# hmc-lair-shark-tracking/auv-sim

Measured on NVIDIA B200. Metric: edge_evals_per_s, higher is better.
Workload: dtype f32

## Files before the change

auv-sim_b200/csrc/edge.cuh:

```cuda
#pragma once
#include "geom.cuh"

#ifndef AUV_EDGE_ONE
#define AUV_EDGE_ONE 0
#endif

namespace auv {

template <typename R> struct SteerParams {
    R d2e, dmax, neg_dmax, freq, min_dist, two_vel;
    R w_diff, o_dist, o_diff, o_vel;
};

template <int G> struct Log2 { static const int v = (G == 32) ? 5 : (G == 16) ? 4 : (G == 8) ? 3 : (G == 4) ? 2 : 1; };

template <typename R, int G, bool FLAT = true> struct GroupScratch {
    R us[FLAT ? 3 * G : 32];
    R wx[G + 1], wy[G + 1];
    unsigned char jmp[FLAT ? Log2<G>::v : 1][FLAT ? 3 * G + 4 : 4];
};

template <typename R> struct EdgeOut {
    R x, y, th, t, len;
    int nwp;
    int n_exp;
    uint32_t ctr;
    int status;
    bool safe;
    R s2; uint32_t cnt; uint64_t mask;
    R self_s2; int self_hab; bool leaf_moved;
};

__device__ __forceinline__ float sinc_small(float h) {
    float z = h * h;
    if (z > 0.25f) {
        float sn, cs;
        Ar<float, false>::sincos(h, &sn, &cs);
        return __fdividef(sn, h);
    }
    float p = fmaf(z, 2.7557319e-6f, -1.9841270e-4f);
    p = fmaf(z, p, 8.3333333e-3f);
    p = fmaf(z, p, -1.6666667e-1f);
    return fmaf(z, p, 1.0f);
}

template <typename R, int G, bool DO_COLLIDE, bool DO_COST, bool WRITE_WP, bool FLAT = false, bool ONE_CHUNK = false, bool GRIDS = false>
__device__ __forceinline__ void eval_edge(const Grp<G> &g, GroupScratch<R, G, FLAT> &sc, const EnvView<R> &env,
                                          const Stream<R> &rng, uint32_t ctr, const SteerParams<R> &sp,
                                          R px, R py, R pth, R pt, R plen, R w3, int n_hab,
                                          R *wp_out, int wp_cap, EdgeOut<R> &out) {
    typedef typename Policy<R>::A A;
    const bool VERIFY = Policy<R>::VERIFY;
    const int LOG = Log2<G>::v;

    R u0 = rng.u(ctr);
    ctr += 1;
    int n_exp = (int)A::floor(uniform_ab<R>((R)0, sp.freq, u0));
    out.n_exp = n_exp;
    out.status = 0;

    R cth = pth, cx = px, cy = py, ct = pt, clen = plen;
    R csin = 0, ccos = 0;
    if (VERIFY) A::sincos(pth, &csin, &ccos);
    int nwp = 1;
    bool hit = false, outside = false, zero_div = false, moved = false, degenerate = false, parent_clear = false, parent_many = false;
    R acc_s2 = 0; uint32_t acc_cnt = 0; uint64_t acc_mask = 0;
    R self_s2 = 0; int self_hab = -1;

    if (DO_COLLIDE) {
        if (g.gl == 0) { sc.wx[G] = px; sc.wy[G] = py; }
        const Cls pcl = env.template classify<GRIDS>(px, py);
        parent_clear = (pcl.code & 4u) != 0u;
        parent_many = (pcl.code & AUV_GRID_CIRC_MANY) != 0u;
        if (VERIFY || !AUV_EDGE_ONE || (pcl.code & AUV_GRID_SLOW)) {
            outside = !point_within_c<R>(env, pcl, px, py);
            if (!parent_clear && !parent_many) hit = point_hits_circles_c<R>(env, pcl, px, py);
        } else outside = point_unsafe_one<R>(env, pcl.code, px, py);
    }

    for (int base = 0; base < n_exp; base += G) {
        const int nact = min(G, n_exp - base);
        const bool act = g.gl < nact;
        R dist = 0, diff = 0, vt = 1;
        bool valid = false;
        if (FLAT) {
    #pragma unroll
            for (int r = 0; r < 3; r++) {
                int s = g.gl + G * r;
                sc.us[s] = (s < 3 * nact) ? rng.u(ctr + (uint32_t)s) : (R)0;
            }
            g.sync();
    #pragma unroll
            for (int r = 0; r < 3; r++) {
                int s = g.gl + G * r;
                int nx = 3 * G;
                if (s <= 3 * G - 3) {
                    R dist = uniform_ab<R>((R)0, sp.d2e, sc.us[s]);
                    R diff = uniform_ab<R>(sp.neg_dmax, sp.dmax, sc.us[s + 1]);
                    nx = s + 2 + (A::fabs(dist) > A::fabs(diff) ? 1 : 0);
                    if (nx > 3 * G) nx = 3 * G;
                }
                sc.jmp[0][s] = (unsigned char)nx;
            }
            if (g.gl == 0) {
    #pragma unroll
                for (int d = 0; d < LOG; d++) sc.jmp[d][3 * G] = (unsigned char)(3 * G);
            }
            g.sync();
    #pragma unroll
            for (int d = 1; d < LOG; d++) {
    #pragma unroll
                for (int r = 0; r < 3; r++) {
                    int s = g.gl + G * r;
                    sc.jmp[d][s] = sc.jmp[d - 1][sc.jmp[d - 1][s]];
                }
                g.sync();
            }
            int o = 0;
    #pragma unroll
            for (int d = 0; d < LOG; d++)
                if ((g.gl >> d) & 1) o = sc.jmp[d][o];
            if (act) {
                dist = uniform_ab<R>((R)0, sp.d2e, sc.us[o]);
                diff = uniform_ab<R>(sp.neg_dmax, sp.dmax, sc.us[o + 1]);
                valid = A::fabs(dist) > A::fabs(diff);
                if (valid) vt = uniform_ab<R>((R)0, sp.two_vel, sc.us[o + 2]);
            }
            int o_end = g.bcast(o + 2 + (valid ? 1 : 0), nact - 1);
            ctr += (uint32_t)o_end;

        } else {
            if (act) {
                const uint32_t p0 = ctr + 3u * (uint32_t)g.gl;
                dist = uniform_ab<R>((R)0, sp.d2e, rng.u(p0));
                diff = uniform_ab<R>(sp.neg_dmax, sp.dmax, rng.u(p0 + 1u));
                valid = A::fabs(dist) > A::fabs(diff);
                if (valid) vt = uniform_ab<R>((R)0, sp.two_vel, rng.u(p0 + 2u));
            }
            ctr += 3u * (uint32_t)nact;
        }
        R phi = 0, radius = 0, chord = 0;
        if (valid) {
            if (VERIFY) {
                R s1 = A::add(dist, diff), s2 = A::sub(dist, diff);
                R den = A::add(-s1, s2);
                R num = A::add(s1, s2);
                if (den == (R)0) zero_div = true;
                radius = A::div(num, den);
                R r2 = A::mul((R)2, radius);
                if (r2 == (R)0) zero_div = true;
                phi = A::div(num, r2);
            } else {
                if (diff == (R)0) zero_div = true;
                phi = -diff;
                chord = dist * sinc_small((float)diff * 0.5f);
            }
            if (vt == (R)0) zero_div = true;
        }
        R th;
        if (VERIFY) th = (R)grp_scan_serial<G>(g, (double)phi, (double)cth);
        else th = grp_scan_incl<G>(g, phi) + cth;
        R dx = 0, dy = 0, movement = 0, dt = 0;
        if (VERIFY) {
            R s1v, c1v;
            A::sincos(th, &s1v, &c1v);
            R s0v = g.up(s1v, 1), c0v = g.up(c1v, 1);
            if (g.gl == 0) { s0v = csin; c0v = ccos; }
            if (valid) {
                dx = A::mul(radius, A::sub(s1v, s0v));
                dy = A::mul(radius, A::add(-c1v, c0v));
                movement = A::sqrt(A::sq2(dx, dy));
                dt = A::div(movement, vt);
            }
            csin = g.bcast(s1v, G - 1); ccos = g.bcast(c1v, G - 1);
        } else {
            if (valid) {
                R sm, cm;
                A::sincos(th - (R)0.5 * phi, &sm, &cm);
                dx = chord * cm; dy = chord * sm;
                movement = chord;
                dt = A::div(movement, vt);
            }
        }
        R x, y, t, len;
        if (VERIFY) {
            x = (R)grp_scan_serial<G>(g, (double)dx, (double)cx);
            y = (R)grp_scan_serial<G>(g, (double)dy, (double)cy);
            t = (R)grp_scan_serial<G>(g, (double)dt, (double)ct);
            len = (R)grp_scan_serial<G>(g, (double)movement, (double)clen);
        } else {
            x = grp_scan_incl<G>(g, dx) + cx;
            y = grp_scan_incl<G>(g, dy) + cy;
            t = grp_scan_incl<G>(g, dt) + ct;
            len = grp_scan_incl<G>(g, movement) + clen;
        }
        const bool is_wp = valid && (movement >= sp.min_dist);
        const unsigned wpm = g.ballot(is_wp);
        const unsigned vm = g.ballot(valid);
        if (vm) moved = true;
        const int last_valid = vm ? 31 - __clz(vm) : -1;

        if (WRITE_WP) {
            if (is_wp) {
                int row = nwp - 1 + __popc(wpm & ((1u << g.gl) - 1u));
                if (row < wp_cap) {
                    R *w = wp_out + 6 * (size_t)row;
                    w[0] = x; w[1] = y; w[2] = th; w[3] = vt; w[4] = t; w[5] = len;
                }
            }
        }
        Cls cl; cl.code = AUV_GRID_ALL_AMBIG | 4u; cl.idx = -1;
        if ((DO_COLLIDE || DO_COST) && (is_wp || g.gl == last_valid)) cl = env.template classify<GRIDS>(x, y);
        if (DO_COLLIDE) {
            bool in = true, h1 = false;
            if (is_wp) {
                if (VERIFY || !AUV_EDGE_ONE) {
                    in = point_within_c<R>(env, cl, x, y);
                    if (!(cl.code & AUV_GRID_CIRC_MANY)) h1 = point_hits_circles_c<R>(env, cl, x, y);
                } else {
                    in = !point_unsafe_one<R>(env, cl.code, x, y);
                    if (__builtin_expect((cl.code & AUV_GRID_SLOW) != 0u, 0)) {
                        in = point_within_c<R>(env, cl, x, y);
                        if (!(cl.code & AUV_GRID_CIRC_MANY)) h1 = point_hits_circles_c<R>(env, cl, x, y);
                    }
                }
            }
            if (g.ballot(!in)) outside = true;
            if (g.ballot(h1)) hit = true;
            const bool circles_needed = g.ballot(is_wp && !(cl.code & 4u) && (cl.code & AUV_GRID_CIRC_MANY)) != 0u ||
                                        (base == 0 && !parent_clear && parent_many);
            if (env.K > 0 && circles_needed && !outside) {
                if (is_wp) { int slot = __popc(wpm & ((1u << g.gl) - 1u)); sc.wx[slot] = x; sc.wy[slot] = y; }
                g.sync();
                const int nw = __popc(wpm);
                bool h = false;
#pragma unroll 1
                for (int k = g.gl; k < env.K; k += G) {
                    R ccx = env.cx[k], ccy = env.cy[k];
                    R q = A::inf();
                    if (base == 0) q = A::sq2(A::sub(sc.wx[G], ccx), A::sub(sc.wy[G], ccy));
#pragma unroll 1
                    for (int j = 0; j < nw; j++) {
                        R qq = A::sq2(A::sub(sc.wx[j], ccx), A::sub(sc.wy[j], ccy));
                        q = qq < q ? qq : q;
                    }
                    if (VERIFY) h = h || (A::sqrt(q) <= env.creff[k]);
                    else h = h || (q <= env.creff2[k]);
                }
                if (g.ballot(h)) hit = true;
                g.sync();
            }
        }
        if (DO_COST) {
            const bool need = is_wp || (g.gl == last_valid);
            Contrib c; c.bin = -1; c.cell = -1; c.hab = -1;
            if (need) c = point_contrib<R>(env, x, y, t, 0xffffffffu, n_hab, cl);
            R ps2 = (R)0;
            if (c.bin >= 0 && c.cell >= 0) ps2 = A::mul(w3, env.probs[(size_t)c.bin * env.C + c.cell]);
            const bool counts = is_wp && c.bin >= 0;
            acc_s2 += grp_sum<G>(g, counts ? ps2 : (R)0);
            unsigned hm = g.ballot(counts && c.hab >= 0);
            acc_cnt += __popc(hm);
            unsigned long long mbits = (counts && c.hab >= 0) ? (1ull << c.hab) : 0ull;
            if (G == 32) {
                const unsigned lo = __reduce_or_sync(0xffffffffu, (unsigned)mbits), hi = __reduce_or_sync(0xffffffffu, (unsigned)(mbits >> 32));
                mbits = ((unsigned long long)hi << 32) | lo;
            } else {
#pragma unroll
                for (int m = G / 2; m > 0; m >>= 1) mbits |= g.xorv(mbits, m);
            }
            acc_mask |= mbits;
            if (last_valid >= 0) {
                self_s2 = g.bcast((c.bin >= 0) ? ps2 : (R)0, last_valid);
                self_hab = g.bcast((c.bin >= 0) ? c.hab : -1, last_valid);
            }
        }
        nwp += __popc(wpm);
        if (last_valid >= 0) {
            cth = g.bcast(th, last_valid); cx = g.bcast(x, last_valid); cy = g.bcast(y, last_valid);
            ct = g.bcast(t, last_valid); clen = g.bcast(len, last_valid);
        }
        g.sync();
        if (g.ballot(zero_div)) {
            if (VERIFY) out.status = 2; else degenerate = true;
            break;
        }
        if (ONE_CHUNK) break;
    }
    if (DO_COLLIDE && n_exp == 0 && env.K > 0 && !parent_clear && parent_many) {
        bool h = false;
#pragma unroll 1
        for (int k = g.gl; k < env.K; k += G) {
            R q = A::sq2(A::sub(px, env.cx[k]), A::sub(py, env.cy[k]));
            if (VERIFY) h = h || (A::sqrt(q) <= env.creff[k]);
            else h = h || (q <= env.creff2[k]);
        }
        if (g.ballot(h)) hit = true;
    }
    if (!rng.consumed_ok(ctr)) out.status = 4;
    out.x = cx; out.y = cy; out.th = cth; out.t = ct; out.len = clen;
    out.nwp = nwp; out.ctr = ctr;
    out.safe = !(hit || outside || degenerate);
    out.s2 = acc_s2; out.cnt = acc_cnt; out.mask = acc_mask;
    out.self_s2 = self_s2; out.self_hab = self_hab; out.leaf_moved = moved;
}

}
```

auv-sim_b200/csrc/env.cuh:

```cuda
#pragma once
#include "common.cuh"

namespace auv {

struct EnvHeader {
    int K, E, H, T, C, NB, NP, NCAND;
    int convex;
    int hot_bytes;
    int total_bytes;
    int off_cx, off_cy, off_cr, off_creff, off_creff2;
    int off_px, off_py;
    int off_hx, off_hy, off_hr, off_hr2;
    int off_b0, off_b1;
    int off_brk, off_piece, off_c1, off_cell;
    int off_probs;
    int off_xb;
    int nxb;
    int off_pfirst;
    int off_grid;
    int gnx, gny;
    int bins_uniform;
    int off_one;
    int pad_;
    double bbox[4];
    double gx0, gy0, gs;
    double bin_s0, bin_w;
    double xb0, xbw;
    double pad2_[2];
};
static_assert(sizeof(EnvHeader) % 16 == 0, "EnvHeader must keep 16-byte alignment of the arrays");

#define AUV_GRID_HAB_NONE 128u
#define AUV_GRID_HAB_AMBIG 192u
#define AUV_GRID_HAB_ONE 64u
#define AUV_GRID_CIRC_MANY (1u << 11)
#define AUV_GRID_HAB_MANY (1u << 12)
#define AUV_GRID_POLY_FULL (1u << 13)
#define AUV_GRID_CIRC_ONE (1u << 14)
#define AUV_GRID_POLY_ONE (1u << 15)
#define AUV_GRID_SLOW (1u << 31)
#define AUV_GRID_ALL_AMBIG ((AUV_GRID_HAB_AMBIG << 3) | AUV_GRID_CIRC_MANY | AUV_GRID_HAB_MANY | AUV_GRID_POLY_FULL | AUV_GRID_SLOW)

struct Cls { unsigned code; int idx; };

template <typename R> struct alignas(8) PFirst { R c1; int v; };

template <typename R> struct alignas(16) One { R x, y, z, w; };

template <typename R> struct EnvView {
    int K, E, H, T, C, NB, NP, convex;
    int gnx, gny, ncell, bins_uniform, nxb;
    R gx0, gy0, ginv, gxo, gyo, bin_s0, bin_w, bin_winv, bin_off, bin_lo, bin_hi, xb0, xbinv, xbo;
    const unsigned *grid;
    const unsigned *grid0s;
    const PFirst<R> *pfirst;
    const One<R> *cone, *pone, *hone;
    const EnvView<R> *shared_self;
    const unsigned short *xb;
    R minx, miny, maxx, maxy;
    const R *cx, *cy, *cr, *creff, *creff2;
    const R *px, *py;
    const R *hx, *hy, *hr, *hr2;
    const R *b0, *b1;
    const R *brk;
    const int *piece;
    const R *c1;
    const int *cell;
    const R *probs;

    __device__ __forceinline__ void bind(const unsigned char *hot, const unsigned char *probs_base) {
        const EnvHeader *h = (const EnvHeader *)hot;
        K = h->K; E = h->E; H = h->H; T = h->T; C = h->C; NB = h->NB; NP = h->NP; convex = h->convex;
        shared_self = nullptr;
        minx = (R)h->bbox[0]; miny = (R)h->bbox[1]; maxx = (R)h->bbox[2]; maxy = (R)h->bbox[3];
        cx = (const R *)(hot + h->off_cx); cy = (const R *)(hot + h->off_cy);
        cr = (const R *)(hot + h->off_cr); creff = (const R *)(hot + h->off_creff);
        creff2 = (const R *)(hot + h->off_creff2);
        px = (const R *)(hot + h->off_px); py = (const R *)(hot + h->off_py);
        hx = (const R *)(hot + h->off_hx); hy = (const R *)(hot + h->off_hy);
        hr = (const R *)(hot + h->off_hr); hr2 = (const R *)(hot + h->off_hr2);
        b0 = (const R *)(hot + h->off_b0); b1 = (const R *)(hot + h->off_b1);
        brk = (const R *)(hot + h->off_brk); piece = (const int *)(hot + h->off_piece);
        c1 = (const R *)(hot + h->off_c1); cell = (const int *)(hot + h->off_cell);
        probs = (const R *)(probs_base + h->off_probs);
        pfirst = (const PFirst<R> *)(hot + h->off_pfirst);
        cone = (const One<R> *)(hot + h->off_one); pone = cone + (K + 1); hone = pone + (E > 0 ? E : 1);
        bin_lo = T > 0 ? b0[0] : (R)1; bin_hi = T > 0 ? b1[T - 1] : (R)0;
    }
    __device__ __forceinline__ void assume_hot_shared(bool probs_too) const {
        __builtin_assume(__isShared(cx)); __builtin_assume(__isShared(cy)); __builtin_assume(__isShared(cr));
        __builtin_assume(__isShared(creff)); __builtin_assume(__isShared(creff2));
        __builtin_assume(__isShared(px)); __builtin_assume(__isShared(py));
        __builtin_assume(__isShared(hx)); __builtin_assume(__isShared(hy)); __builtin_assume(__isShared(hr));
        __builtin_assume(__isShared(hr2)); __builtin_assume(__isShared(b0)); __builtin_assume(__isShared(b1));
        __builtin_assume(__isShared(brk)); __builtin_assume(__isShared(piece)); __builtin_assume(__isShared(c1));
        __builtin_assume(__isShared(cell)); __builtin_assume(__isShared(pfirst)); __builtin_assume(__isShared(xb));
        __builtin_assume(__isShared(cone)); __builtin_assume(__isShared(pone)); __builtin_assume(__isShared(hone));
        if (probs_too) __builtin_assume(__isShared(probs));
    }
    __device__ __forceinline__ void bind_grid(const unsigned char *blob_global, const unsigned char *hot) {
        const EnvHeader *h = (const EnvHeader *)hot;
        gnx = h->gnx; gny = h->gny; bins_uniform = h->bins_uniform; nxb = h->nxb;
        xb0 = (R)h->xb0; xbinv = (R)(1.0 / h->xbw); xbo = (R)(-h->xb0 / h->xbw); xb = (const unsigned short *)(hot + h->off_xb);
        gx0 = (R)h->gx0; gy0 = (R)h->gy0; ginv = (R)(1.0 / h->gs);
        gxo = (R)(-h->gx0 / h->gs); gyo = (R)(-h->gy0 / h->gs);
        bin_s0 = (R)h->bin_s0; bin_w = (R)h->bin_w; bin_winv = (R)(1.0 / h->bin_w); bin_off = (R)(-h->bin_s0 / h->bin_w);
        grid = (const unsigned *)(blob_global + h->off_grid);
        grid0s = nullptr;
        ncell = gnx * gny;
    }
    template <bool GRIDS = false>
    __device__ __forceinline__ Cls classify(R x, R y) const {
        Cls c;
        int ix, iy;
        if (sizeof(R) == 4) {
            const float fx = fmaf((float)x, (float)ginv, (float)gxo), fy = fmaf((float)y, (float)ginv, (float)gyo);
            ix = __float_as_int(__fadd_rd(fx, 8388608.f)) - 0x4B000000;
            iy = __float_as_int(__fadd_rd(fy, 8388608.f)) - 0x4B000000;
        } else {
            const R fx = (x - gx0) * ginv, fy = (y - gy0) * ginv;
            const bool in = fx >= (R)0 && fy >= (R)0 && fx < (R)gnx && fy < (R)gny;
            ix = in ? (int)fx : -1; iy = in ? (int)fy : -1;
        }
        if (!((unsigned)ix < (unsigned)gnx && (unsigned)iy < (unsigned)gny)) {
            c.code = gnx > 0 ? (((AUV_GRID_HAB_AMBIG << 3) | AUV_GRID_HAB_MANY | AUV_GRID_CIRC_MANY | AUV_GRID_POLY_FULL) | 2u) : AUV_GRID_ALL_AMBIG;
            c.idx = -1; return c;
        }
        c.idx = iy * gnx + ix;
        c.code = GRIDS ? grid0s[c.idx] : __ldg(grid + c.idx);
        return c;
    }
    __device__ __forceinline__ unsigned word1(const Cls &c) const { return __ldg(grid + ncell + c.idx); }
    __device__ __forceinline__ unsigned word2(const Cls &c) const { return __ldg(grid + 2 * ncell + c.idx); }
};

__device__ __forceinline__ uint32_t smem_u32(const void *p) {
    return (uint32_t)__cvta_generic_to_shared(p);
}
__device__ __forceinline__ void mbar_init(uint64_t *bar, int count) {
    asm volatile("mbarrier.init.shared::cta.b64 [%0], %1;" ::"r"(smem_u32(bar)), "r"(count));
    asm volatile("fence.mbarrier_init.release.cluster;" ::: "memory");
}
__device__ __forceinline__ void mbar_expect_tx(uint64_t *bar, uint32_t bytes) {
    asm volatile("mbarrier.arrive.expect_tx.shared::cta.b64 _, [%0], %1;" ::"r"(smem_u32(bar)), "r"(bytes)
                 : "memory");
}
__device__ __forceinline__ void tma_bulk_g2s(void *dst, const void *src, uint32_t bytes, uint64_t *bar) {
    asm volatile(
        "cp.async.bulk.shared::cluster.global.mbarrier::complete_tx::bytes [%0], [%1], %2, [%3];" ::"r"(
            smem_u32(dst)),
        "l"(src), "r"(bytes), "r"(smem_u32(bar))
        : "memory");
}
__device__ __forceinline__ void mbar_wait(uint64_t *bar, uint32_t phase) {
    asm volatile(
        "{\n"
        ".reg .pred p;\n"
        "WAIT_%=:\n"
        "mbarrier.try_wait.parity.shared::cta.b64 p, [%0], %1;\n"
        "@p bra DONE_%=;\n"
        "bra WAIT_%=;\n"
        "DONE_%=:\n"
        "}\n" ::"r"(smem_u32(bar)),
        "r"(phase)
        : "memory");
}

__device__ __forceinline__ void stage_env_tma(unsigned char *smem_dst, const unsigned char *blob,
                                              int bytes, uint64_t *bar) {
    if (threadIdx.x == 0) mbar_init(bar, 1);
    __syncthreads();
    if (threadIdx.x == 0) {
        mbar_expect_tx(bar, (uint32_t)bytes);
        for (int o = 0; o < bytes; o += 65536) {
            int n = bytes - o < 65536 ? bytes - o : 65536;
            tma_bulk_g2s(smem_dst + o, blob + o, (uint32_t)n, bar);
        }
    }
    mbar_wait(bar, 0);
}

struct EnvStagePlan { int bytes; int probs_staged; };

}
```

auv-sim_b200/csrc/plan.cu:

```cuda
#include <stdlib.h>
#include "plan_common.cuh"
#include "dubins.cuh"

#ifndef AUV_PLAN_PREFETCH
#define AUV_PLAN_PREFETCH 0
#endif

namespace auv {

#define AUV_LAUNCH_CHECK2()                                                                 \
    do {                                                                                    \
        g_launches++;                                                                       \
        cudaError_t e_ = cudaGetLastError();                                                \
        if (e_ != cudaSuccess)                                                              \
            return set_err(AUVRRT_ERR_CUDA, "%s:%d launch: %s", __FILE__, __LINE__,         \
                           cudaGetErrorString(e_));                                         \
    } while (0)

#ifndef AUV_PLAN_THREADS32
#define AUV_PLAN_THREADS32 896
#endif
#ifndef AUV_PLAN_MINB32
#define AUV_PLAN_MINB32 (896 / AUV_PLAN_THREADS32)
#endif
template <typename R, int G> struct PlanCta {
    static const int T = (sizeof(R) == 4 && G == 32) ? AUV_PLAN_THREADS32 : 128, MINB = (sizeof(R) == 4 && G == 32) ? AUV_PLAN_MINB32 : 7;
};

struct WsLayout {
    size_t slot_bytes;
    size_t rows, xy, pool, next, head, tail, count;
};

template <typename R> static WsLayout make_layout(int cap, int nb, int nchunks) {
    WsLayout L;
    size_t o = 0;
    auto take = [&](size_t bytes) { size_t r = o; o += (bytes + 127) & ~(size_t)127; return r; };
    L.rows = take(sizeof(NodeRow<R>) * (size_t)cap);
    L.xy = take(2 * sizeof(R) * (size_t)cap);
    L.pool = take(4 * 32 * (size_t)nchunks); L.next = take(4 * (size_t)nchunks);
    L.head = take(4 * (size_t)(nb + 2)); L.tail = take(4 * (size_t)(nb + 2)); L.count = take(4 * (size_t)(nb + 2));
    L.slot_bytes = o;
    return L;
}

template <typename R> struct Tree {
    NodeRow<R> *row;
    R *nx, *ny;
    int *pool, *next, *head, *tail, *count;
    __device__ __forceinline__ void bind(unsigned char *b, const WsLayout &L, int cap) {
        row = (NodeRow<R> *)(b + L.rows);
        nx = (R *)(b + L.xy); ny = nx + cap;
        pool = (int *)(b + L.pool); next = (int *)(b + L.next);
        head = (int *)(b + L.head); tail = (int *)(b + L.tail); count = (int *)(b + L.count);
    }
};

template <typename R> struct DubinsEdge {
    bool ok;
    bool safe;
    R x, y, th, t, len;
    R s2; uint32_t cnt; unsigned long long mask;
    R self_s2; int self_hab;
};
template <typename R>
__device__ __forceinline__ void dubins_edge_eval(const EnvView<R> &env, const PlanP<R> &P, R px, R py, R pth, R pt, R plen,
                                                 R sx, R sy, R sth, bool do_tests, R *rows, int room, DubinsEdge<R> &e) {
    typedef typename Policy<R>::A A;
    e.ok = false; e.safe = false; e.x = px; e.y = py; e.th = pth; e.t = pt; e.len = plen;
    e.s2 = 0; e.cnt = 0; e.mask = 0ull; e.self_s2 = 0; e.self_hab = -1;
    const DubinsPath<R> d = dubins_shortest<R>(px, py, pth, sx, sy, sth, P.rho);
    if (d.word < 0) return;
    e.ok = true;
    const R s_end = d.length < P.eta ? d.length : P.eta;
    const R step = A::div(s_end, (R)(P.W - 1));
    DubinsSampler<R> smp;
    smp.init(d, px, py, pth, P.rho);
    bool bad = false;
    if (do_tests) {
        const Cls pcl = env.classify(px, py);
        bad = point_unsafe_c<R>(env, pcl, px, py);
    }
#pragma unroll 1
    for (int k = 1; k < P.W; k++) {
        const R sk = A::mul((R)k, step);
        R x, y, th;
        smp.at(sk, x, y, th);
        const R t = A::add(pt, A::div(sk, P.vel)), len = A::add(plen, sk);
        if (do_tests) {
            const Cls cl = env.classify(x, y);
            bad = bad || point_unsafe_c<R>(env, cl, x, y);
            const Contrib c = point_contrib<R>(env, x, y, t, 0xffffffffu, env.H, cl);
            const R ps2 = (c.bin >= 0 && c.cell >= 0) ? A::mul(P.w3, env.probs[(size_t)c.bin * env.C + c.cell]) : (R)0;
            if (c.bin >= 0) {
                e.s2 = A::add(e.s2, ps2);
                if (c.hab >= 0) { e.cnt++; e.mask |= 1ull << c.hab; }
            }
            e.self_s2 = c.bin >= 0 ? ps2 : (R)0; e.self_hab = c.bin >= 0 ? c.hab : -1;
        }
        if (rows && k - 1 < room) {
            R *w = rows + 6 * (size_t)(k - 1);
            w[0] = x; w[1] = y; w[2] = th; w[3] = P.vel; w[4] = t; w[5] = len;
        }
        e.x = x; e.y = y; e.th = th; e.t = t; e.len = len;
    }
    e.safe = !bad;
}
template <typename R>
__device__ __forceinline__ void dubins_sample_at(const EnvView<R> &env, const Stream<R> &rng, uint32_t ctr, R &sx, R &sy, R &sth) {
    sx = uniform_ab<R>(env.minx, env.maxx, rng.u(ctr));
    sy = uniform_ab<R>(env.miny, env.maxy, rng.u(ctr + 1u));
    sth = uniform_ab<R>((R)-3.141592653589793, (R)3.141592653589793, rng.u(ctr + 2u));
}

#define AUV_BINS_SMEM 128
template <typename R> struct BestPlan { R c0, c1, c2, len, t; int node, iter; };
template <typename R, int G, bool BS, int MODE, bool ONE>
__global__ void __launch_bounds__(PlanCta<R, G>::T, sizeof(R) == 4 ? PlanCta<R, G>::MINB : (PlanCta<R, G>::MINB + 1) / 2)
k_plan(const unsigned char *blob, int hot_bytes, int total_bytes, int stage_mode, const R *starts,
       const uint64_t *seeds, long long Q, PlanP<R> P, WsLayout L, unsigned char *ws, unsigned long long *qcounter,
       auvrrt_plan_record_t *records, uint32_t *chain_out, R *path_out, auvrrt_plan_trace_t tr) {
    typedef typename Policy<R>::A A;
    const bool VERIFY = Policy<R>::VERIFY;
    const int pick_mode = MODE >= 0 ? MODE : P.mode;
    extern __shared__ __align__(16) unsigned char smem[];
    const int PLAN_THREADS = PlanCta<R, G>::T;
    __shared__ GroupScratch<R, G, false> scratch[PlanCta<R, G>::T / G];
    __shared__ BestPlan<R> best_s[PlanCta<R, G>::T / G];
    __shared__ unsigned short binmeta[BS ? PlanCta<R, G>::T / G : 1][3][BS ? AUV_BINS_SMEM : 1];
    EnvView<R> env;
    {
        if (stage_mode == 0) { env.bind(blob, blob); env.bind_grid(blob, blob); }
        else if (stage_mode == 3) {
            uint64_t *bar = (uint64_t *)smem;
            const EnvHeader *gh = (const EnvHeader *)blob;
            const int plane = (gh->gnx * gh->gny * 4 + 15) & ~15;
            if (threadIdx.x == 0) mbar_init(bar, 1);
            __syncthreads();
            if (threadIdx.x == 0) {
                mbar_expect_tx(bar, (uint32_t)(total_bytes + plane));
                for (int o = 0; o < total_bytes; o += 65536) tma_bulk_g2s(smem + 16 + o, blob + o, (uint32_t)(total_bytes - o < 65536 ? total_bytes - o : 65536), bar);
                const unsigned char *gsrc = blob + gh->off_grid;
                for (int o = 0; o < plane; o += 65536) tma_bulk_g2s(smem + 16 + total_bytes + o, gsrc + o, (uint32_t)(plane - o < 65536 ? plane - o : 65536), bar);
            }
            mbar_wait(bar, 0);
            env.bind(smem + 16, smem + 16);
            env.bind_grid(blob, smem + 16);
            env.grid0s = (const unsigned *)(smem + 16 + total_bytes);
            __builtin_assume(__isShared(env.grid0s));
        } else {
            uint64_t *bar = (uint64_t *)smem;
            stage_env_tma(smem + 16, blob, stage_mode == 2 ? total_bytes : hot_bytes, bar);
            env.bind(smem + 16, stage_mode == 2 ? smem + 16 : blob);
            env.bind_grid(blob, smem + 16);
        }
        if (ONE) env.assume_hot_shared(PlanCta<R, G>::T >= 896);
    }
    Grp<G> g;
    GroupScratch<R, G, false> &sc = scratch[threadIdx.x / G];
    const int slot = blockIdx.x * (PLAN_THREADS / G) + threadIdx.x / G;
    Tree<R> T;
    T.bind(ws + (size_t)slot * L.slot_bytes, L, P.cap);
    unsigned short *s_count = binmeta[BS ? threadIdx.x / G : 0][0], *s_head = binmeta[BS ? threadIdx.x / G : 0][1],
                   *s_tail = binmeta[BS ? threadIdx.x / G : 0][2];
#define BIN_COUNT(b) (BS ? (int)s_count[b] : T.count[b])
#define BIN_HEAD(b) (BS ? (int)s_head[b] : T.head[b])
#define BIN_TAIL(b) (BS ? (int)s_tail[b] : T.tail[b])
#define SET_BIN_COUNT(b, v) do { if (BS) s_count[b] = (unsigned short)(v); else T.count[b] = (v); } while (0)
#define SET_BIN_HEAD(b, v) do { if (BS) s_head[b] = (unsigned short)(v); else T.head[b] = (v); } while (0)
#define SET_BIN_TAIL(b, v) do { if (BS) s_tail[b] = (unsigned short)(v); else T.tail[b] = (v); } while (0)

    for (;;) {
        long long q = 0;
        if (g.gl == 0) q = (long long)atomicAdd(qcounter, 1ull);
        q = g.bcast(q, 0);
        if (q >= Q) break;

        Stream<R> rng;
        rng.key = stream_key(seeds[q]); rng.ext = nullptr; rng.n_ext = 0;
        const R sx = starts[5 * q], sy = starts[5 * q + 1], sth = starts[5 * q + 2], st = starts[5 * q + 3],
                slen = starts[5 * q + 4];
        for (int b = g.gl; b < P.nb + 2; b += G) SET_BIN_COUNT(b, 0);
        if (g.gl == 0) {
            NodeRow<R> r0;
            r0.x = sx; r0.y = sy; r0.th = sth; r0.t = st; r0.len = slen;
            r0.parent = -1; r0.ctr = 0; r0.s2 = (R)0; r0.cnt = 0; r0.mask = 0ull; r0.born = 0;
            Contrib c = point_contrib<R>(env, sx, sy, st, 0xffffffffu, env.H, env.classify(sx, sy));
            r0.self_s2 = (c.bin >= 0 && c.cell >= 0) ? A::mul(P.w3, env.probs[(size_t)c.bin * env.C + c.cell]) : (R)0;
            r0.self_hab = c.bin >= 0 ? c.hab : -1;
            T.row[0] = r0;
            if (pick_mode == 1 || pick_mode == 3) { T.nx[0] = sx; T.ny[0] = sy; }
        }
        g.sync();
        if (g.gl == 0) { SET_BIN_HEAD(1, 0); SET_BIN_TAIL(1, 0); SET_BIN_COUNT(1, 1); T.pool[0] = 0; T.next[0] = -1; }
        g.sync();
        int n_nodes = 1, n_chunks = 1;
        uint32_t ctr = 0, upos_mark = 0;
        int status = AUVRRT_ST_OK;
        int n_cost_evals = 0;
        unsigned n_waypoints = 0, n_prims = 0;
        R best_total = A::inf();
        if (g.gl == 0) { BestPlan<R> b0; b0.c0 = b0.c1 = b0.c2 = b0.len = b0.t = (R)0; b0.node = -1; b0.iter = -1; best_s[threadIdx.x / G] = b0; }
        int it = 0;
        int guard = 0;
        const int guard_max = (int)min(64LL * P.I + 1024, 2147483647LL);

        while (it < P.I && guard++ < guard_max) {
            int parent;
            if (pick_mode == 3) {
                const uint32_t ctr0 = ctr;
                R smx, smy, smth;
                dubins_sample_at<R>(env, rng, ctr, smx, smy, smth);
                ctr += 4;
                int *near = (int *)sc.us;
                R bq = A::inf(), bs = A::inf();
                int bi = 0x7fffffff, nlist = 0;
                for (int i0 = 0; i0 < n_nodes; i0 += G) {
                    const int i = i0 + g.gl;
                    bool in = false;
                    if (i < n_nodes) {
                        const R qq = A::sq2(A::sub(smx, T.nx[i]), A::sub(smy, T.ny[i]));
                        if (qq < bq) {
                            if (VERIFY) { R sd = A::sqrt(qq); if (sd < bs) { bs = sd; bi = i; } }
                            else { bs = qq; bi = i; }
                            bq = qq;
                        }
                        in = VERIFY ? (A::sqrt(qq) <= P.near_r) : (qq <= P.near_r2);
                    }
                    const unsigned m = g.ballot(in);
                    if (in) {
                        const int pos = nlist + __popc(m & ((1u << g.gl) - 1u));
                        if (pos < G) near[pos] = i;
                    }
                    nlist += __popc(m);
                }
                nlist = min(nlist, G);
#pragma unroll
                for (int mm = G / 2; mm > 0; mm >>= 1) {
                    R os = g.xorv(bs, mm);
                    int oi = g.xorv(bi, mm);
                    if (os < bs || (os == bs && oi < bi)) { bs = os; bi = oi; }
                }
                const int nearest = bi;
                g.sync();
                if (T.row[nearest].t > P.max_traj) { upos_mark = ctr; continue; }
                int pn = nlist;
                for (int j = g.gl; j < nlist; j += G) if (near[j] == nearest) pn = j;
#pragma unroll
                for (int mm = G / 2; mm > 0; mm >>= 1) pn = min(pn, g.xorv(pn, mm));
                const int ncand = min(G, 1 + nlist - (pn < nlist ? 1 : 0));
                int pidx = -1;
                if (g.gl == 0) pidx = nearest;
                else if (g.gl < ncand) { const int j = g.gl - 1; pidx = near[j < pn ? j : j + 1]; }
                g.sync();
                DubinsEdge<R> de;
                de.ok = false; de.safe = false; de.x = de.y = de.th = de.t = de.len = 0; de.s2 = 0; de.cnt = 0; de.mask = 0ull;
                de.self_s2 = 0; de.self_hab = -1;
                NodeRow<R> pr;
                pr.s2 = 0; pr.self_s2 = 0; pr.cnt = 0; pr.mask = 0ull; pr.self_hab = -1; pr.t = 0;
                if (pidx >= 0) {
                    pr = T.row[pidx];
                    if (!(pr.t > P.max_traj))
                        dubins_edge_eval<R>(env, P, pr.x, pr.y, pr.th, pr.t, pr.len, smx, smy, smth, true, nullptr, 0, de);
                }
                n_waypoints += (unsigned)(P.W * __popc(g.ballot(de.ok)));
                R pre_s2 = 0, c0 = 0, c1 = 0, c2 = 0, total = A::inf();
                uint32_t pre_cnt = 0; unsigned long long pre_mask = 0;
                if (de.ok && de.safe) {
                    const int ph = pr.self_hab;
                    pre_s2 = A::add(A::add(pr.s2, pr.self_s2), de.s2);
                    pre_cnt = pr.cnt + (ph >= 0 ? 1u : 0u) + de.cnt;
                    pre_mask = pr.mask | (ph >= 0 ? (1ull << ph) : 0ull) | de.mask;
                    const uint32_t cnt = pre_cnt + (de.self_hab >= 0 ? 1u : 0u);
                    const unsigned long long mk = pre_mask | (de.self_hab >= 0 ? (1ull << de.self_hab) : 0ull);
                    c1 = A::mul(P.w2, (R)cnt);
                    c2 = A::add(pre_s2, de.self_s2);
                    if (de.t > (R)0) { c1 = A::div(c1, de.t); c2 = A::div(c2, de.t); }
                    if (env.H != 0) c0 = A::div(A::mul(P.w1, (R)__popcll(mk)), (R)env.H);
                    total = py_sum3p<R>(c0, c1, c2);
                }
                R bt = total; int bp = (de.ok && de.safe) ? pidx : 0x7fffffff;
#pragma unroll
                for (int mm = G / 2; mm > 0; mm >>= 1) {
                    R ot = g.xorv(bt, mm);
                    int op = g.xorv(bp, mm);
                    if (ot < bt || (ot == bt && op < bp)) { bt = ot; bp = op; }
                }
                const bool any_safe = bp != 0x7fffffff;
                const unsigned wm = g.ballot(any_safe && pidx == bp && de.ok && de.safe);
                const int bl = wm ? __ffs(wm) - 1 : 0;
                const R nx_ = g.bcast(de.x, bl), ny_ = g.bcast(de.y, bl), nth_ = g.bcast(de.th, bl), nt_ = g.bcast(de.t, bl),
                        nlen_ = g.bcast(de.len, bl);
                if (P.trace && g.gl == 0) {
                    size_t r = (size_t)q * P.I + it;
                    tr.parent[r] = any_safe ? bp : -1; tr.safe[r] = any_safe ? 1 : 0; tr.nwp[r] = P.W; tr.upos[r] = upos_mark;
                    R *lf = (R *)tr.leaf + 5 * r;
                    lf[0] = nx_; lf[1] = ny_; lf[2] = nth_; lf[3] = nt_; lf[4] = nlen_;
                }
                if (any_safe) {
                    const int id = n_nodes++;
                    if (g.gl == bl) {
                        NodeRow<R> nr;
                        nr.x = de.x; nr.y = de.y; nr.th = de.th; nr.t = de.t; nr.len = de.len; nr.parent = bp; nr.ctr = ctr0;
                        nr.s2 = pre_s2; nr.cnt = pre_cnt; nr.mask = pre_mask; nr.self_s2 = de.self_s2; nr.self_hab = de.self_hab;
                        nr.born = it;
                        T.row[id] = nr;
                        T.nx[id] = de.x; T.ny[id] = de.y;
                    }
                    if (nt_ >= P.horizon) {
                        n_cost_evals++;
                        if (bt < best_total) {
                            best_total = bt;
                            if (g.gl == bl) {
                                BestPlan<R> b; b.c0 = c0; b.c1 = c1; b.c2 = c2; b.len = de.len; b.t = de.t; b.node = id; b.iter = it;
                                best_s[threadIdx.x / G] = b;
                            }
                        }
                    }
                }
                g.sync();
                it++;
                upos_mark = ctr;
                continue;
            }
            if (pick_mode == 0) {
                int ran_bin = 0, bincnt = 0;
                bool kerr = false;
                for (;;) {
                    R u = rng.u(ctr + (uint32_t)g.gl);
                    int rb = (int)uniform_ab<R>((R)1, (R)(P.nb + 1), u);
                    bool ke = rb > P.nb || rb < 1;
                    int cn = ke ? 0 : BIN_COUNT(rb);
                    unsigned m = g.ballot(ke || cn > 0);
                    if (m) {
                        int f = __ffs(m) - 1;
                        ran_bin = g.bcast(rb, f); bincnt = g.bcast(cn, f); kerr = g.bcast(ke ? 1 : 0, f) != 0;
                        ctr += (uint32_t)f + 1u;
                        break;
                    }
                    ctr += G;
                }
                if (kerr) { status = AUVRRT_ST_KEY_ERROR; break; }
                g.sync();
                R u = rng.u(ctr);
                ctr += 1;
                int idx = (int)uniform_ab<R>((R)0, (R)bincnt, u);
                if (idx >= bincnt) { status = AUVRRT_ST_KEY_ERROR; break; }
                int ch = BIN_HEAD(ran_bin);
#pragma unroll 1
                for (int hop = idx >> 5; hop > 0; hop--) ch = T.next[ch];
                parent = T.pool[ch * 32 + (idx & 31)];
            } else if (pick_mode == 2) {
                const R ran_time = uniform_ab<R>((R)0, P.ran_time_max, rng.u(ctr));
                ctr += 1;
                parent = closest_mps_time<R>(T.row, n_nodes, ran_time, P.plan_dt);
                if (T.row[parent].t > P.max_traj) continue;
            } else {
                R rx = uniform_ab<R>(env.minx, env.maxx, rng.u(ctr));
                R ry = uniform_ab<R>(env.miny, env.maxy, rng.u(ctr + 1));
                ctr += 4;
                R bq = A::inf(), bs = A::inf();
                int bi = 0x7fffffff;
                for (int i = g.gl; i < n_nodes; i += G) {
                    R qq = A::sq2(A::sub(rx, T.nx[i]), A::sub(ry, T.ny[i]));
                    if (qq < bq) {
                        if (VERIFY) { R s = A::sqrt(qq); if (s < bs) { bs = s; bi = i; } }
                        else { bs = qq; bi = i; }
                        bq = qq;
                    }
                }
#pragma unroll
                for (int m = G / 2; m > 0; m >>= 1) {
                    R os = g.xorv(bs, m);
                    int oi = g.xorv(bi, m);
                    if (os < bs || (os == bs && oi < bi)) { bs = os; bi = oi; }
                }
                parent = bi;
                if (T.row[parent].t > P.max_traj) continue;
            }
            const NodeRow<R> pr = T.row[parent];
            const R ppx = pr.x, ppy = pr.y, ppth = pr.th, ppt = pr.t, pplen = pr.len;
            const uint32_t ctr0 = ctr;
#if AUV_PLAN_PREFETCH
            int spec_parent = -1;
            if (ONE && BS && pick_mode == 0) {
                const int n_exp_now = (int)A::floor(uniform_ab<R>((R)0, P.sp.freq, rng.u(ctr)));
                const uint32_t cn0 = ctr + 1u + 3u * (uint32_t)(n_exp_now > 0 ? n_exp_now : 0);
                const int rb = (int)uniform_ab<R>((R)1, (R)(P.nb + 1), rng.u(cn0 + (uint32_t)g.gl));
                const int cn = (rb >= 1 && rb <= P.nb) ? (int)s_count[rb] : 0;
                const unsigned m = g.ballot(cn > 0);
                if (m) {
                    const int f = __ffs(m) - 1;
                    const int sb = g.bcast(rb, f), sc_ = g.bcast(cn, f);
                    const int idx = (int)uniform_ab<R>((R)0, (R)sc_, rng.u(cn0 + (uint32_t)f + 1u));
                    if (idx < 32 && idx < sc_) spec_parent = T.pool[(int)s_head[sb] * 32 + idx];
                }
            }
#endif
            EdgeOut<R> o;
            eval_edge<R, G, true, true, false, false, ONE, ONE && (PlanCta<R, G>::T >= 896)>(g, sc, env, rng, ctr, P.sp, ppx, ppy, ppth, ppt, pplen, P.w3, env.H,
                                                           nullptr, 0, o);
#if AUV_PLAN_PREFETCH
            if (ONE && BS && pick_mode == 0 && spec_parent >= 0 && g.gl < 2)
                asm volatile("prefetch.global.L1 [%0];" ::"l"((const char *)&T.row[spec_parent] + 32 * g.gl));
#endif
            ctr = o.ctr;
            n_waypoints += o.nwp; n_prims += o.n_exp;
            if (P.trace && g.gl == 0) {
                size_t r = (size_t)q * P.I + it;
                tr.parent[r] = parent; tr.safe[r] = o.safe ? 1 : 0; tr.nwp[r] = o.nwp; tr.upos[r] = upos_mark;
                R *lf = (R *)tr.leaf + 5 * r;
                lf[0] = o.x; lf[1] = o.y; lf[2] = o.th; lf[3] = o.t; lf[4] = o.len;
            }
            if (o.status != 0) { status = o.status; break; }
            if (o.safe) {
                const int id = n_nodes++;
                R pre_s2 = 0, self_s2n = 0;
                uint32_t pre_cnt = 0; unsigned long long pre_mask = 0; int self_habn = -1;
                if (g.gl == 0) {
                    const int ph = pr.self_hab;
                    pre_s2 = A::add(A::add(pr.s2, pr.self_s2), o.s2);
                    pre_cnt = pr.cnt + (ph >= 0 ? 1u : 0u) + o.cnt;
                    pre_mask = pr.mask | (ph >= 0 ? (1ull << ph) : 0ull) | o.mask;
                    self_s2n = o.leaf_moved ? o.self_s2 : pr.self_s2;
                    self_habn = o.leaf_moved ? o.self_hab : ph;
                    NodeRow<R> nr;
                    nr.x = o.x; nr.y = o.y; nr.th = o.th; nr.t = o.t; nr.len = o.len; nr.parent = parent; nr.ctr = ctr0;
                    nr.s2 = pre_s2; nr.cnt = pre_cnt; nr.mask = pre_mask; nr.self_s2 = self_s2n; nr.self_hab = self_habn;
                    nr.born = it;
                    T.row[id] = nr;
                    if (pick_mode == 1 || pick_mode == 3) { T.nx[id] = o.x; T.ny[id] = o.y; }
                }
                if (pick_mode != 2) {
                    R fd = floordiv_pos<R>(o.t, P.bin_interval);
                    R fidx = fd + (R)1;
                    R curr_bin = A::mul(fidx, P.bin_interval);
                    int bidx = -1; bool reset = false;
                    if (curr_bin > P.max_traj) {
                        if (fidx >= (R)1 && fidx <= (R)P.nb) { bidx = (int)fidx; reset = true; }
                    } else {
                        if (fidx >= (R)1 && fidx <= (R)P.nb) bidx = (int)fidx; else status = AUVRRT_ST_KEY_ERROR;
                    }
                    if (bidx >= 0) {
                        const int c_old = g.bcast(g.gl == 0 ? BIN_COUNT(bidx) : 0, 0);
                        const bool reuse_head = reset && c_old > 0;
                        const int c = reset ? 0 : c_old;
                        const bool alloc = ((c & 31) == 0) && !reuse_head;
                        const int nc = n_chunks;
                        if (alloc) n_chunks++;
                        if (g.gl == 0) {
                            int tl = reuse_head ? BIN_HEAD(bidx) : BIN_TAIL(bidx);
                            if (alloc) {
                                T.next[nc] = -1;
                                if (c == 0) SET_BIN_HEAD(bidx, nc); else T.next[tl] = nc;
                                tl = nc;
                            }
                            SET_BIN_TAIL(bidx, tl);
                            T.pool[tl * 32 + (c & 31)] = id;
                            SET_BIN_COUNT(bidx, c + 1);
                        }
                    }
                }
                status = g.bcast(status, 0);
                if (status != AUVRRT_ST_OK) break;
                if (o.t >= P.horizon) {
                    R tot_s2 = 0, c0 = 0, c1 = 0, c2 = 0, total = 0;
                    if (g.gl == 0) {
                        uint32_t cnt = pre_cnt + (self_habn >= 0 ? 1u : 0u);
                        unsigned long long mk = pre_mask | (self_habn >= 0 ? (1ull << self_habn) : 0ull);
                        tot_s2 = A::add(pre_s2, self_s2n);
                        c1 = A::mul(P.w2, (R)cnt);
                        c2 = tot_s2;
                        if (o.t > (R)0) { c1 = A::div(c1, o.t); c2 = A::div(c2, o.t); }
                        if (env.H != 0) c0 = A::div(A::mul(P.w1, (R)__popcll(mk)), (R)env.H);
                        total = py_sum3p<R>(c0, c1, c2);
                    }
                    total = g.bcast(total, 0);
                    n_cost_evals++;
                    if (total < best_total) {
                        best_total = total;
                        if (g.gl == 0) {
                            BestPlan<R> b; b.c0 = c0; b.c1 = c1; b.c2 = c2; b.len = o.len; b.t = o.t; b.node = id; b.iter = it;
                            best_s[threadIdx.x / G] = b;
                        }
                    }
                }
                g.sync();
            }
            it++;
            upos_mark = ctr;
        }
        g.sync();
        const BestPlan<R> best = best_s[threadIdx.x / G];
        const int best_node = best.node, best_iter = best.iter;
        const R best_c[4] = {best_total, best.c0, best.c1, best.c2}, best_len = best.len, best_t = best.t;
        if (status == AUVRRT_ST_OK && best_node < 0) status = AUVRRT_ST_NO_PATH;
        int depth = 0, n_path = 0;
        if (best_node < 0 && chain_out)
            for (int k = g.gl; k < P.chain_cap; k += G) chain_out[(size_t)q * P.chain_cap + k] = 0u;
        if (best_node >= 0) {
            for (int n = best_node; T.row[n].parent >= 0; n = T.row[n].parent) depth++;
            uint32_t *chain = chain_out ? chain_out + (size_t)q * P.chain_cap : nullptr;
            if (depth > P.chain_cap && chain) { if (status == AUVRRT_ST_OK) status = AUVRRT_ST_OVERFLOW; }
            if (chain && g.gl == 0) {
                int n = best_node;
                for (int k = depth - 1; k >= 0; k--) { if (k < P.chain_cap) chain[k] = (uint32_t)n; n = T.row[n].parent; }
            }
            g.sync();
            if (path_out && P.path_cap > 0 && chain && depth <= P.chain_cap) {
                R *rows = path_out + (size_t)q * P.path_cap * 6;
                for (int e = 0; e < depth; e++) {
                    const int id = (int)chain[e];
                    const NodeRow<R> pn = T.row[T.row[id].parent];
                    if (g.gl == 0 && n_path < P.path_cap) {
                        R *w = rows + 6 * (size_t)n_path;
                        w[0] = pn.x; w[1] = pn.y; w[2] = pn.th; w[3] = (pick_mode == 3 && pn.parent >= 0) ? P.vel : (R)0;
                        w[4] = pn.t; w[5] = pn.len;
                    }
                    n_path++;
                    int room = P.path_cap - n_path; if (room < 0) room = 0;
                    if (pick_mode == 3) {
                        if (g.gl == 0) {
                            R smx, smy, smth;
                            dubins_sample_at<R>(env, rng, T.row[id].ctr, smx, smy, smth);
                            DubinsEdge<R> de;
                            dubins_edge_eval<R>(env, P, pn.x, pn.y, pn.th, pn.t, pn.len, smx, smy, smth, false,
                                                rows + 6 * (size_t)(n_path < P.path_cap ? n_path : 0), room, de);
                        }
                        n_path += P.W - 1;
                        continue;
                    }
                    EdgeOut<R> o;
                    eval_edge<R, G, false, false, true>(g, sc, env, rng, T.row[id].ctr, P.sp, pn.x, pn.y, pn.th,
                                                        pn.t, pn.len, (R)0, 0,
                                                        rows + 6 * (size_t)(n_path < P.path_cap ? n_path : 0), room, o);
                    n_path += o.nwp - 1;
                }
                if (g.gl == 0 && n_path < P.path_cap) {
                    R *w = rows + 6 * (size_t)n_path;
                    const NodeRow<R> bn = T.row[best_node];
                    w[0] = bn.x; w[1] = bn.y; w[2] = bn.th; w[3] = (pick_mode == 3 && bn.parent >= 0) ? P.vel : (R)0;
                    w[4] = bn.t; w[5] = bn.len;
                }
                n_path++;
                if (n_path > P.path_cap && status == AUVRRT_ST_OK) status = AUVRRT_ST_OVERFLOW;
            }
            g.sync();
            if (chain && g.gl == 0)
                for (int k = 0; k < depth && k < P.chain_cap; k++) chain[k] = T.row[chain[k]].ctr;
            if (chain) for (int k = depth + g.gl; k < P.chain_cap; k += G) chain[k] = 0u;
        }
        if (g.gl == 0) {
            auvrrt_plan_record_t rec;
            rec.status = status; rec.n_nodes = n_nodes; rec.best_node = best_node; rec.best_iter = best_iter;
            rec.depth = depth; rec.n_path = n_path; rec.n_cost_evals = n_cost_evals;
            rec.n_waypoints = (int32_t)n_waypoints; rec.n_uniforms = (long long)ctr; rec.n_primitives = (long long)n_prims;
            rec.cost[0] = best_node >= 0 ? (double)best_c[0] : 0.0; rec.cost[1] = (double)best_c[1];
            rec.cost[2] = (double)best_c[2]; rec.cost[3] = (double)best_c[3];
            rec.path_length = (double)best_len; rec.t_leaf = (double)best_t;
            records[q] = rec;
        }
        g.sync();
    }
}

template <typename R, int G>
__global__ void __launch_bounds__(128)
k_materialize(const unsigned char *blob, const R *starts, const uint64_t *seeds, const uint32_t *chain,
              const int32_t *depth, long long Q, PlanP<R> P, R *path_out, int32_t *n_path_out) {
    __shared__ GroupScratch<R, G, false> scratch[128 / G];
    EnvView<R> env;
    env.bind(blob, blob);
    env.bind_grid(blob, blob);
    Grp<G> g;
    GroupScratch<R, G, false> &sc = scratch[threadIdx.x / G];
    const long long groups = (long long)gridDim.x * (128 / G);
    for (long long q = blockIdx.x * (long long)(128 / G) + threadIdx.x / G; q < Q; q += groups) {
        Stream<R> rng;
        rng.key = stream_key(seeds[q]); rng.ext = nullptr; rng.n_ext = 0;
        R x = starts[5 * q], y = starts[5 * q + 1], th = starts[5 * q + 2], t = starts[5 * q + 3], len = starts[5 * q + 4];
        R *rows = path_out + (size_t)q * P.path_cap * 6;
        int n_path = 0;
        const int d = depth[q];
        for (int e = 0; e < d; e++) {
            if (g.gl == 0 && n_path < P.path_cap) {
                R *w = rows + 6 * (size_t)n_path;
                w[0] = x; w[1] = y; w[2] = th; w[3] = (P.mode == 3 && e > 0) ? P.vel : (R)0; w[4] = t; w[5] = len;
            }
            n_path++;
            int room = P.path_cap - n_path; if (room < 0) room = 0;
            if (P.mode == 3) {
                R smx, smy, smth;
                dubins_sample_at<R>(env, rng, chain[(size_t)q * P.chain_cap + e], smx, smy, smth);
                DubinsEdge<R> de;
                dubins_edge_eval<R>(env, P, x, y, th, t, len, smx, smy, smth, false,
                                    g.gl == 0 ? rows + 6 * (size_t)(n_path < P.path_cap ? n_path : 0) : nullptr, room, de);
                n_path += P.W - 1;
                x = de.x; y = de.y; th = de.th; t = de.t; len = de.len;
                continue;
            }
            EdgeOut<R> o;
            eval_edge<R, G, false, false, true>(g, sc, env, rng, chain[(size_t)q * P.chain_cap + e], P.sp, x, y, th, t,
                                                len, (R)0, 0, rows + 6 * (size_t)(n_path < P.path_cap ? n_path : 0),
                                                room, o);
            n_path += o.nwp - 1;
            x = o.x; y = o.y; th = o.th; t = o.t; len = o.len;
        }
        if (d >= 0) {
            if (g.gl == 0 && n_path < P.path_cap) {
                R *w = rows + 6 * (size_t)n_path;
                w[0] = x; w[1] = y; w[2] = th; w[3] = (P.mode == 3 && d > 0) ? P.vel : (R)0; w[4] = t; w[5] = len;
            }
            n_path++;
        }
        if (g.gl == 0) n_path_out[q] = n_path;
    }
}

template <typename R, int G, bool BS, int MODE, bool ONE> static int plan_geometry(const auvrrt_env *env, int *grid, int *smem, int *stage_mode) {
    EnvBlob<R> b = env_blob<R>(env);
    int budget = sizeof(R) == 4 ? (PlanCta<R, G>::T >= 896 ? 96 * 1024 : 24 * 1024) : 110 * 1024;
    if (const char *ev = getenv("AUVRRT_PLAN_STAGE_KB")) budget = atoi(ev) * 1024;
    if (const char *ev = getenv("AUVRRT_PLAN_BUDGET_KB")) budget = atoi(ev) * 1024;
    int sm = 16, mode = 0;
    if (b.total_bytes + 16 <= budget) { sm = b.total_bytes + 16; mode = 2; }
    else if (b.hot_bytes + 16 <= budget) { sm = b.hot_bytes + 16; mode = 1; }
    if (ONE && PlanCta<R, G>::T >= 896) {
        const EnvHeader &hd = sizeof(R) == 4 ? env->h32 : env->h64;
        sm = b.total_bytes + 16 + ((hd.gnx * hd.gny * 4 + 15) & ~15); mode = 3;
    }
    AUV_CUDA(cudaFuncSetAttribute(k_plan<R, G, BS, MODE, ONE>, cudaFuncAttributeMaxDynamicSharedMemorySize, sm));
    int per_sm = 0;
    AUV_CUDA(cudaOccupancyMaxActiveBlocksPerMultiprocessor(&per_sm, k_plan<R, G, BS, MODE, ONE>, PlanCta<R, G>::T, sm));
    if (per_sm < 1) return set_err(AUVRRT_ERR_CUDA, "plan: kernel does not fit on an SM (smem %d)", sm);
    int nsm = 0, dev = 0;
    AUV_CUDA(cudaGetDevice(&dev));
    AUV_CUDA(cudaDeviceGetAttribute(&nsm, cudaDevAttrMultiProcessorCount, dev));
    *grid = nsm * per_sm; *smem = sm; *stage_mode = mode;
    return AUVRRT_OK;
}

template <typename R, int G, bool BS, int MODE, bool ONE>
static int launch_plan_gb(const auvrrt_env *env, const R *starts, const uint64_t *seeds, int64_t Q,
                         const auvrrt_plan_params_t *p, void *workspace, int64_t workspace_bytes,
                         auvrrt_plan_record_t *records, uint32_t *chain, R *path, const auvrrt_plan_trace_t *trace,
                         cudaStream_t s, int64_t *need_bytes) {
    PlanP<R> P;
    int rc = make_planp<R>(env, p, &P);
    if (rc) return rc;
    int grid, smem, mode;
    rc = plan_geometry<R, G, BS, MODE, ONE>(env, &grid, &smem, &mode);
    if (rc) return rc;
    WsLayout L = make_layout<R>(P.cap, P.nb, P.nchunks);
    const int gpc = PlanCta<R, G>::T / G;
    int64_t need = 256 + (int64_t)grid * gpc * (int64_t)L.slot_bytes;
    if (need_bytes) { *need_bytes = need; return AUVRRT_OK; }
    if (Q <= 0) return AUVRRT_OK;
    if (workspace_bytes < need) return set_err(AUVRRT_ERR_ARG, "plan: workspace too small (%lld < %lld)", (long long)workspace_bytes, (long long)need);
    if (P.trace && !trace) return set_err(AUVRRT_ERR_ARG, "plan: trace requested without trace buffers");
    int64_t blocks = (Q + gpc - 1) / gpc;
    if (blocks < grid) grid = (int)blocks;
    AUV_CUDA(cudaMemsetAsync(workspace, 0, 256, s));
    auvrrt_plan_trace_t tr;
    if (trace) tr = *trace; else { tr.parent = nullptr; tr.safe = nullptr; tr.nwp = nullptr; tr.leaf = nullptr; tr.upos = nullptr; }
    EnvBlob<R> b = env_blob<R>(env);
    k_plan<R, G, BS, MODE, ONE><<<grid, PlanCta<R, G>::T, smem, s>>>(b.blob, b.hot_bytes, b.total_bytes, mode, starts, seeds, (long long)Q, P, L,
                                                  (unsigned char *)workspace + 256, (unsigned long long *)workspace,
                                                  records, chain, path, tr);
    AUV_LAUNCH_CHECK2();
    return AUVRRT_OK;
}

template <typename R, int G>
static int launch_plan_g(const auvrrt_env *env, const R *starts, const uint64_t *seeds, int64_t Q,
                         const auvrrt_plan_params_t *p, void *workspace, int64_t workspace_bytes,
                         auvrrt_plan_record_t *records, uint32_t *chain, R *path, const auvrrt_plan_trace_t *trace,
                         cudaStream_t s, int64_t *need_bytes) {
    const double nb = ceil(p->max_traj_time / p->bin_interval);
    const bool bs = nb + 2 <= AUV_BINS_SMEM && p->iterations < 65000 && !getenv("AUVRRT_PLAN_BINS_GLOBAL");
#define AUV_PLAN_ARGS env, starts, seeds, Q, p, workspace, workspace_bytes, records, chain, path, trace, s, need_bytes
    if constexpr (sizeof(R) == 4) {
        if (p->mode == 0 && !getenv("AUVRRT_PLAN_GENERIC")) {
            const bool fits = PlanCta<R, G>::T >= 896
                                  ? (env->h32.gnx > 0 && env->h32.total_bytes + 16 + env->h32.gnx * env->h32.gny * 4 + 16 <= 180 * 1024)
                                  : env->h32.hot_bytes + 16 <= 24 * 1024;
            if (p->freq <= (double)G && bs && fits && !getenv("AUVRRT_PLAN_STAGE_KB"))
                return launch_plan_gb<R, G, true, 0, true>(AUV_PLAN_ARGS);
            return bs ? launch_plan_gb<R, G, true, 0, false>(AUV_PLAN_ARGS) : launch_plan_gb<R, G, false, 0, false>(AUV_PLAN_ARGS);
        }
    }
    return bs ? launch_plan_gb<R, G, true, -1, false>(AUV_PLAN_ARGS) : launch_plan_gb<R, G, false, -1, false>(AUV_PLAN_ARGS);
#undef AUV_PLAN_ARGS
}

template <typename R>
int launch_plan(const auvrrt_env *env, const R *starts, const uint64_t *seeds, int64_t Q,
                const auvrrt_plan_params_t *p, void *workspace, int64_t workspace_bytes,
                auvrrt_plan_record_t *records, uint32_t *chain, R *path, const auvrrt_plan_trace_t *trace,
                cudaStream_t s) {
    int G = p->group ? p->group : ((Q >= 32768 && !(path && p->path_cap > 0) && p->mode != 3) ? 1 : 32);
    if (G == 1 && p->mode == 3) return set_err(AUVRRT_ERR_UNSUPPORTED, "plan: mode 3 evaluates one candidate parent per lane; group must be 32, 16 or 8");
    if (G == 1) {
        if (path && p->path_cap > 0) return set_err(AUVRRT_ERR_UNSUPPORTED, "plan: group 1 (thread per tree) writes no paths; use auvrrt_materialize");
        return launch_plan_tpt<R>(env, starts, seeds, Q, p, workspace, workspace_bytes, records, chain, trace, s, nullptr);
    }
    if (G == 32) return launch_plan_g<R, 32>(env, starts, seeds, Q, p, workspace, workspace_bytes, records, chain, path, trace, s, nullptr);
    if (G == 16) return launch_plan_g<R, 16>(env, starts, seeds, Q, p, workspace, workspace_bytes, records, chain, path, trace, s, nullptr);
    if (G == 8) return launch_plan_g<R, 8>(env, starts, seeds, Q, p, workspace, workspace_bytes, records, chain, path, trace, s, nullptr);
    return set_err(AUVRRT_ERR_ARG, "plan: group must be 32, 16, 8 or 1");
}
template <typename R>
int64_t plan_workspace_bytes(const auvrrt_env *env, const auvrrt_plan_params_t *p, int64_t Q) {
    int64_t need = -1;
    int rc;
    const int G = p->group ? p->group : 32;
    if (G == 1) rc = launch_plan_tpt<R>(env, nullptr, nullptr, Q, p, nullptr, 0, nullptr, nullptr, nullptr, 0, &need);
    else if (G == 32) rc = launch_plan_g<R, 32>(env, nullptr, nullptr, 0, p, nullptr, 0, nullptr, nullptr, nullptr, nullptr, 0, &need);
    else if (G == 16) rc = launch_plan_g<R, 16>(env, nullptr, nullptr, 0, p, nullptr, 0, nullptr, nullptr, nullptr, nullptr, 0, &need);
    else if (G == 8) rc = launch_plan_g<R, 8>(env, nullptr, nullptr, 0, p, nullptr, 0, nullptr, nullptr, nullptr, nullptr, 0, &need);
    else { set_err(AUVRRT_ERR_ARG, "plan: group must be 32, 16, 8 or 1"); return -1; }
    if (rc) return -1;
    if (p->group == 0 && p->mode != 3 && (Q <= 0 || Q >= 32768)) {
        int64_t tpt = -1;
        if (launch_plan_tpt<R>(env, nullptr, nullptr, Q, p, nullptr, 0, nullptr, nullptr, nullptr, 0, &tpt)) return -1;
        if (tpt > need) need = tpt;
    }
    return need;
}
template int launch_plan<float>(const auvrrt_env *, const float *, const uint64_t *, int64_t, const auvrrt_plan_params_t *,
                                void *, int64_t, auvrrt_plan_record_t *, uint32_t *, float *, const auvrrt_plan_trace_t *, cudaStream_t);
template int launch_plan<double>(const auvrrt_env *, const double *, const uint64_t *, int64_t, const auvrrt_plan_params_t *,
                                 void *, int64_t, auvrrt_plan_record_t *, uint32_t *, double *, const auvrrt_plan_trace_t *, cudaStream_t);
template int64_t plan_workspace_bytes<float>(const auvrrt_env *, const auvrrt_plan_params_t *, int64_t);
template int64_t plan_workspace_bytes<double>(const auvrrt_env *, const auvrrt_plan_params_t *, int64_t);

template <typename R>
int launch_materialize(const auvrrt_env *env, const R *starts, const uint64_t *seeds, const uint32_t *chain,
                       const int32_t *depth, int64_t Q, const auvrrt_plan_params_t *p, R *path, int32_t *n_path,
                       cudaStream_t s) {
    if (Q <= 0) return AUVRRT_OK;
    PlanP<R> P;
    int rc = make_planp<R>(env, p, &P);
    if (rc) return rc;
    const int G = p->group ? p->group : 32;
    if (G == 1) {
        if (p->mode == 3) return set_err(AUVRRT_ERR_UNSUPPORTED, "materialize: mode 3 has no thread-per-tree plans");
        return launch_materialize_tpt<R>(env, starts, seeds, chain, depth, Q, P, path, n_path, s);
    }
    int64_t blocks = (Q * G + 127) / 128;
    if (blocks > AUV_SMS * 8) blocks = AUV_SMS * 8;
    const unsigned char *blob = env_blob<R>(env).blob;
    if (G == 32) k_materialize<R, 32><<<(unsigned)blocks, 128, 0, s>>>(blob, starts, seeds, chain, depth, (long long)Q, P, path, n_path);
    else if (G == 16) k_materialize<R, 16><<<(unsigned)blocks, 128, 0, s>>>(blob, starts, seeds, chain, depth, (long long)Q, P, path, n_path);
    else if (G == 8) k_materialize<R, 8><<<(unsigned)blocks, 128, 0, s>>>(blob, starts, seeds, chain, depth, (long long)Q, P, path, n_path);
    else return set_err(AUVRRT_ERR_ARG, "materialize: group must be 32, 16, 8 or 1");
    AUV_LAUNCH_CHECK2();
    return AUVRRT_OK;
}
template int launch_materialize<float>(const auvrrt_env *, const float *, const uint64_t *, const uint32_t *, const int32_t *,
                                       int64_t, const auvrrt_plan_params_t *, float *, int32_t *, cudaStream_t);
template int launch_materialize<double>(const auvrrt_env *, const double *, const uint64_t *, const uint32_t *, const int32_t *,
                                        int64_t, const auvrrt_plan_params_t *, double *, int32_t *, cudaStream_t);

}
```

Before: 1.132 billion.

## Fold parent-point collision check into one-chunk edge pass and pass env view by grid constant

In the one-chunk edge path, the separate parent classify and collision check are dropped, and the parent point is checked by the last lane inside the main per-chunk collision step. The host now precomputes the environment view and passes it as a grid constant, so the kernel only rebases pointers into the staged shared copy instead of parsing the header. Per-group shared scratch, best-plan and bin arrays are merged into one struct. Tree pointers are computed on demand, the RNG key setup is moved later, and broadcasts in the cost computation are removed. The aim is fewer serial classify calls, fewer registers and less setup work. The risk is a lane conflict when the last lane is also an active sample lane, and a tighter host predicate for enabling one-chunk mode.

Measured after the change: 1.283 billion (median of 6 runs). 1.13x the previous value.

```diff
diff --git a/auv-sim_b200/csrc/edge.cuh b/auv-sim_b200/csrc/edge.cuh
--- a/auv-sim_b200/csrc/edge.cuh
+++ b/auv-sim_b200/csrc/edge.cuh
@@ -69,6 +69,8 @@
 
     if (DO_COLLIDE) {
         if (g.gl == 0) { sc.wx[G] = px; sc.wy[G] = py; }
+    }
+    if (DO_COLLIDE && !ONE_CHUNK) {
         const Cls pcl = env.template classify<GRIDS>(px, py);
         parent_clear = (pcl.code & 4u) != 0u;
         parent_many = (pcl.code & AUV_GRID_CIRC_MANY) != 0u;
@@ -78,8 +80,8 @@
         } else outside = point_unsafe_one<R>(env, pcl.code, px, py);
     }
 
-    for (int base = 0; base < n_exp; base += G) {
-        const int nact = min(G, n_exp - base);
+    for (int base = 0; ONE_CHUNK ? base == 0 : base < n_exp; base += G) {
+        const int nact = ONE_CHUNK ? max(min(G, n_exp), 0) : min(G, n_exp - base);
         const bool act = g.gl < nact;
         R dist = 0, diff = 0, vt = 1;
         bool valid = false;
@@ -209,26 +211,28 @@
                 }
             }
         }
+        const bool pl = ONE_CHUNK && DO_COLLIDE && g.gl == G - 1;
+        const R tx = pl ? px : x, ty = pl ? py : y;
         Cls cl; cl.code = AUV_GRID_ALL_AMBIG | 4u; cl.idx = -1;
-        if ((DO_COLLIDE || DO_COST) && (is_wp || g.gl == last_valid)) cl = env.template classify<GRIDS>(x, y);
+        if ((DO_COLLIDE || DO_COST) && (is_wp || g.gl == last_valid || pl)) cl = env.template classify<GRIDS>(tx, ty);
         if (DO_COLLIDE) {
             bool in = true, h1 = false;
-            if (is_wp) {
+            if (is_wp || pl) {
                 if (VERIFY || !AUV_EDGE_ONE) {
-                    in = point_within_c<R>(env, cl, x, y);
-                    if (!(cl.code & AUV_GRID_CIRC_MANY)) h1 = point_hits_circles_c<R>(env, cl, x, y);
+                    in = point_within_c<R>(env, cl, tx, ty);
+                    if (!(cl.code & AUV_GRID_CIRC_MANY)) h1 = point_hits_circles_c<R>(env, cl, tx, ty);
                 } else {
-                    in = !point_unsafe_one<R>(env, cl.code, x, y);
+                    in = !point_unsafe_one<R>(env, cl.code, tx, ty);
                     if (__builtin_expect((cl.code & AUV_GRID_SLOW) != 0u, 0)) {
-                        in = point_within_c<R>(env, cl, x, y);
-                        if (!(cl.code & AUV_GRID_CIRC_MANY)) h1 = point_hits_circles_c<R>(env, cl, x, y);
+                        in = point_within_c<R>(env, cl, tx, ty);
+                        if (!(cl.code & AUV_GRID_CIRC_MANY)) h1 = point_hits_circles_c<R>(env, cl, tx, ty);
                     }
                 }
             }
             if (g.ballot(!in)) outside = true;
             if (g.ballot(h1)) hit = true;
-            const bool circles_needed = g.ballot(is_wp && !(cl.code & 4u) && (cl.code & AUV_GRID_CIRC_MANY)) != 0u ||
-                                        (base == 0 && !parent_clear && parent_many);
+            const bool circles_needed = g.ballot((is_wp || (pl && n_exp >= 0)) && !(cl.code & 4u) && (cl.code & AUV_GRID_CIRC_MANY)) != 0u ||
+                                        (!ONE_CHUNK && base == 0 && !parent_clear && parent_many);
             if (env.K > 0 && circles_needed && !outside) {
                 if (is_wp) { int slot = __popc(wpm & ((1u << g.gl) - 1u)); sc.wx[slot] = x; sc.wy[slot] = y; }
                 g.sync();
@@ -287,7 +291,7 @@
         }
         if (ONE_CHUNK) break;
     }
-    if (DO_COLLIDE && n_exp == 0 && env.K > 0 && !parent_clear && parent_many) {
+    if (!ONE_CHUNK && DO_COLLIDE && n_exp == 0 && env.K > 0 && !parent_clear && parent_many) {
         bool h = false;
 #pragma unroll 1
         for (int k = g.gl; k < env.K; k += G) {
diff --git a/auv-sim_b200/csrc/env.cuh b/auv-sim_b200/csrc/env.cuh
--- a/auv-sim_b200/csrc/env.cuh
+++ b/auv-sim_b200/csrc/env.cuh
@@ -68,24 +68,34 @@
     const int *cell;
     const R *probs;
 
+    __host__ __device__ __forceinline__ void bind_header(const EnvHeader &h, const unsigned char *hot, const unsigned char *probs_base) {
+        K = h.K; E = h.E; H = h.H; T = h.T; C = h.C; NB = h.NB; NP = h.NP; convex = h.convex;
+        shared_self = nullptr;
+        minx = (R)h.bbox[0]; miny = (R)h.bbox[1]; maxx = (R)h.bbox[2]; maxy = (R)h.bbox[3];
+        cx = (const R *)(hot + h.off_cx); cy = (const R *)(hot + h.off_cy);
+        cr = (const R *)(hot + h.off_cr); creff = (const R *)(hot + h.off_creff);
+        creff2 = (const R *)(hot + h.off_creff2);
+        px = (const R *)(hot + h.off_px); py = (const R *)(hot + h.off_py);
+        hx = (const R *)(hot + h.off_hx); hy = (const R *)(hot + h.off_hy);
+        hr = (const R *)(hot + h.off_hr); hr2 = (const R *)(hot + h.off_hr2);
+        b0 = (const R *)(hot + h.off_b0); b1 = (const R *)(hot + h.off_b1);
+        brk = (const R *)(hot + h.off_brk); piece = (const int *)(hot + h.off_piece);
+        c1 = (const R *)(hot + h.off_c1); cell = (const int *)(hot + h.off_cell);
+        probs = (const R *)(probs_base + h.off_probs);
+        pfirst = (const PFirst<R> *)(hot + h.off_pfirst);
+        cone = (const One<R> *)(hot + h.off_one); pone = cone + (K + 1); hone = pone + (E > 0 ? E : 1);
+    }
     __device__ __forceinline__ void bind(const unsigned char *hot, const unsigned char *probs_base) {
-        const EnvHeader *h = (const EnvHeader *)hot;
-        K = h->K; E = h->E; H = h->H; T = h->T; C = h->C; NB = h->NB; NP = h->NP; convex = h->convex;
-        shared_self = nullptr;
-        minx = (R)h->bbox[0]; miny = (R)h->bbox[1]; maxx = (R)h->bbox[2]; maxy = (R)h->bbox[3];
-        cx = (const R *)(hot + h->off_cx); cy = (const R *)(hot + h->off_cy);
-        cr = (const R *)(hot + h->off_cr); creff = (const R *)(hot + h->off_creff);
-        creff2 = (const R *)(hot + h->off_creff2);
-        px = (const R *)(hot + h->off_px); py = (const R *)(hot + h->off_py);
-        hx = (const R *)(hot + h->off_hx); hy = (const R *)(hot + h->off_hy);
-        hr = (const R *)(hot + h->off_hr); hr2 = (const R *)(hot + h->off_hr2);
-        b0 = (const R *)(hot + h->off_b0); b1 = (const R *)(hot + h->off_b1);
-        brk = (const R *)(hot + h->off_brk); piece = (const int *)(hot + h->off_piece);
-        c1 = (const R *)(hot + h->off_c1); cell = (const int *)(hot + h->off_cell);
-        probs = (const R *)(probs_base + h->off_probs);
-        pfirst = (const PFirst<R> *)(hot + h->off_pfirst);
-        cone = (const One<R> *)(hot + h->off_one); pone = cone + (K + 1); hone = pone + (E > 0 ? E : 1);
+        bind_header(*(const EnvHeader *)hot, hot, probs_base);
         bin_lo = T > 0 ? b0[0] : (R)1; bin_hi = T > 0 ? b1[T - 1] : (R)0;
+    }
+    __device__ __forceinline__ void move_staged(const unsigned char *from, const unsigned char *to) {
+#define AUV_MOVE(p) p = (decltype(p))(to + ((const unsigned char *)(p) - from))
+        AUV_MOVE(cx); AUV_MOVE(cy); AUV_MOVE(cr); AUV_MOVE(creff); AUV_MOVE(creff2); AUV_MOVE(px); AUV_MOVE(py);
+        AUV_MOVE(hx); AUV_MOVE(hy); AUV_MOVE(hr); AUV_MOVE(hr2); AUV_MOVE(b0); AUV_MOVE(b1);
+        AUV_MOVE(brk); AUV_MOVE(piece); AUV_MOVE(c1); AUV_MOVE(cell); AUV_MOVE(probs); AUV_MOVE(pfirst);
+        AUV_MOVE(cone); AUV_MOVE(pone); AUV_MOVE(hone); AUV_MOVE(xb);
+#undef AUV_MOVE
     }
     __device__ __forceinline__ void assume_hot_shared(bool probs_too) const {
         __builtin_assume(__isShared(cx)); __builtin_assume(__isShared(cy)); __builtin_assume(__isShared(cr));
@@ -98,16 +108,18 @@
         __builtin_assume(__isShared(cone)); __builtin_assume(__isShared(pone)); __builtin_assume(__isShared(hone));
         if (probs_too) __builtin_assume(__isShared(probs));
     }
-    __device__ __forceinline__ void bind_grid(const unsigned char *blob_global, const unsigned char *hot) {
-        const EnvHeader *h = (const EnvHeader *)hot;
-        gnx = h->gnx; gny = h->gny; bins_uniform = h->bins_uniform; nxb = h->nxb;
-        xb0 = (R)h->xb0; xbinv = (R)(1.0 / h->xbw); xbo = (R)(-h->xb0 / h->xbw); xb = (const unsigned short *)(hot + h->off_xb);
-        gx0 = (R)h->gx0; gy0 = (R)h->gy0; ginv = (R)(1.0 / h->gs);
-        gxo = (R)(-h->gx0 / h->gs); gyo = (R)(-h->gy0 / h->gs);
-        bin_s0 = (R)h->bin_s0; bin_w = (R)h->bin_w; bin_winv = (R)(1.0 / h->bin_w); bin_off = (R)(-h->bin_s0 / h->bin_w);
-        grid = (const unsigned *)(blob_global + h->off_grid);
+    __host__ __device__ __forceinline__ void bind_grid_header(const EnvHeader &h, const unsigned char *blob_global, const unsigned char *hot) {
+        gnx = h.gnx; gny = h.gny; bins_uniform = h.bins_uniform; nxb = h.nxb;
+        xb0 = (R)h.xb0; xbinv = (R)(1.0 / h.xbw); xbo = (R)(-h.xb0 / h.xbw); xb = (const unsigned short *)(hot + h.off_xb);
+        gx0 = (R)h.gx0; gy0 = (R)h.gy0; ginv = (R)(1.0 / h.gs);
+        gxo = (R)(-h.gx0 / h.gs); gyo = (R)(-h.gy0 / h.gs);
+        bin_s0 = (R)h.bin_s0; bin_w = (R)h.bin_w; bin_winv = (R)(1.0 / h.bin_w); bin_off = (R)(-h.bin_s0 / h.bin_w);
+        grid = (const unsigned *)(blob_global + h.off_grid);
         grid0s = nullptr;
         ncell = gnx * gny;
+    }
+    __device__ __forceinline__ void bind_grid(const unsigned char *blob_global, const unsigned char *hot) {
+        bind_grid_header(*(const EnvHeader *)hot, blob_global, hot);
     }
     template <bool GRIDS = false>
     __device__ __forceinline__ Cls classify(R x, R y) const {
diff --git a/auv-sim_b200/csrc/plan.cu b/auv-sim_b200/csrc/plan.cu
--- a/auv-sim_b200/csrc/plan.cu
+++ b/auv-sim_b200/csrc/plan.cu
@@ -45,15 +45,17 @@
 }
 
 template <typename R> struct Tree {
-    NodeRow<R> *row;
-    R *nx, *ny;
-    int *pool, *next, *head, *tail, *count;
-    __device__ __forceinline__ void bind(unsigned char *b, const WsLayout &L, int cap) {
-        row = (NodeRow<R> *)(b + L.rows);
-        nx = (R *)(b + L.xy); ny = nx + cap;
-        pool = (int *)(b + L.pool); next = (int *)(b + L.next);
-        head = (int *)(b + L.head); tail = (int *)(b + L.tail); count = (int *)(b + L.count);
-    }
+    unsigned char *b;
+    const WsLayout &L;
+    int cap;
+    __device__ __forceinline__ NodeRow<R> *row() const { return (NodeRow<R> *)(b + L.rows); }
+    __device__ __forceinline__ R *nx() const { return (R *)(b + L.xy); }
+    __device__ __forceinline__ R *ny() const { return nx() + cap; }
+    __device__ __forceinline__ int *pool() const { return (int *)(b + L.pool); }
+    __device__ __forceinline__ int *next() const { return (int *)(b + L.next); }
+    __device__ __forceinline__ int *head() const { return (int *)(b + L.head); }
+    __device__ __forceinline__ int *tail() const { return (int *)(b + L.tail); }
+    __device__ __forceinline__ int *count() const { return (int *)(b + L.count); }
 };
 
 template <typename R> struct DubinsEdge {
@@ -115,23 +117,26 @@
 
 #define AUV_BINS_SMEM 128
 template <typename R> struct BestPlan { R c0, c1, c2, len, t; int node, iter; };
+template <typename R, int G, bool BS> struct GroupSmem {
+    GroupScratch<R, G, false> sc;
+    BestPlan<R> best;
+    unsigned short bins[3][BS ? AUV_BINS_SMEM : 1];
+};
 template <typename R, int G, bool BS, int MODE, bool ONE>
 __global__ void __launch_bounds__(PlanCta<R, G>::T, sizeof(R) == 4 ? PlanCta<R, G>::MINB : (PlanCta<R, G>::MINB + 1) / 2)
-k_plan(const unsigned char *blob, int hot_bytes, int total_bytes, int stage_mode, const R *starts,
-       const uint64_t *seeds, long long Q, PlanP<R> P, WsLayout L, unsigned char *ws, unsigned long long *qcounter,
-       auvrrt_plan_record_t *records, uint32_t *chain_out, R *path_out, auvrrt_plan_trace_t tr) {
+k_plan(const unsigned char *blob, int hot_bytes, int total_bytes, int stage_mode, const __grid_constant__ EnvView<R> envp,
+       const R *starts, const uint64_t *seeds, long long Q, PlanP<R> P, const __grid_constant__ WsLayout L,
+       unsigned char *ws, unsigned long long *qcounter, auvrrt_plan_record_t *records, uint32_t *chain_out, R *path_out,
+       auvrrt_plan_trace_t tr) {
     typedef typename Policy<R>::A A;
     const bool VERIFY = Policy<R>::VERIFY;
     const int pick_mode = MODE >= 0 ? MODE : P.mode;
     extern __shared__ __align__(16) unsigned char smem[];
     const int PLAN_THREADS = PlanCta<R, G>::T;
-    __shared__ GroupScratch<R, G, false> scratch[PlanCta<R, G>::T / G];
-    __shared__ BestPlan<R> best_s[PlanCta<R, G>::T / G];
-    __shared__ unsigned short binmeta[BS ? PlanCta<R, G>::T / G : 1][3][BS ? AUV_BINS_SMEM : 1];
+    __shared__ GroupSmem<R, G, BS> groups[PlanCta<R, G>::T / G];
     EnvView<R> env;
     {
-        if (stage_mode == 0) { env.bind(blob, blob); env.bind_grid(blob, blob); }
-        else if (stage_mode == 3) {
+        if ((ONE && PlanCta<R, G>::T >= 896) || stage_mode == 3) {
             uint64_t *bar = (uint64_t *)smem;
             const EnvHeader *gh = (const EnvHeader *)blob;
             const int plane = (gh->gnx * gh->gny * 4 + 15) & ~15;
@@ -144,10 +149,14 @@
                 for (int o = 0; o < plane; o += 65536) tma_bulk_g2s(smem + 16 + total_bytes + o, gsrc + o, (uint32_t)(plane - o < 65536 ? plane - o : 65536), bar);
             }
             mbar_wait(bar, 0);
-            env.bind(smem + 16, smem + 16);
-            env.bind_grid(blob, smem + 16);
-            env.grid0s = (const unsigned *)(smem + 16 + total_bytes);
-            __builtin_assume(__isShared(env.grid0s));
+            uint32_t staged = smem_u32(smem + 16);
+            asm volatile("" : "+r"(staged));
+            const unsigned char *sp = (const unsigned char *)__cvta_shared_to_generic(staged);
+            env = envp;
+            env.move_staged(blob, sp);
+            env.grid0s = (const unsigned *)(sp + total_bytes);
+        } else if (stage_mode == 0) {
+            env.bind(blob, blob); env.bind_grid(blob, blob);
         } else {
             uint64_t *bar = (uint64_t *)smem;
             stage_env_tma(smem + 16, blob, stage_mode == 2 ? total_bytes : hot_bytes, bar);
@@ -157,18 +166,19 @@
         if (ONE) env.assume_hot_shared(PlanCta<R, G>::T >= 896);
     }
     Grp<G> g;
-    GroupScratch<R, G, false> &sc = scratch[threadIdx.x / G];
-    const int slot = blockIdx.x * (PLAN_THREADS / G) + threadIdx.x / G;
-    Tree<R> T;
-    T.bind(ws + (size_t)slot * L.slot_bytes, L, P.cap);
-    unsigned short *s_count = binmeta[BS ? threadIdx.x / G : 0][0], *s_head = binmeta[BS ? threadIdx.x / G : 0][1],
-                   *s_tail = binmeta[BS ? threadIdx.x / G : 0][2];
-#define BIN_COUNT(b) (BS ? (int)s_count[b] : T.count[b])
-#define BIN_HEAD(b) (BS ? (int)s_head[b] : T.head[b])
-#define BIN_TAIL(b) (BS ? (int)s_tail[b] : T.tail[b])
-#define SET_BIN_COUNT(b, v) do { if (BS) s_count[b] = (unsigned short)(v); else T.count[b] = (v); } while (0)
-#define SET_BIN_HEAD(b, v) do { if (BS) s_head[b] = (unsigned short)(v); else T.head[b] = (v); } while (0)
-#define SET_BIN_TAIL(b, v) do { if (BS) s_tail[b] = (unsigned short)(v); else T.tail[b] = (v); } while (0)
+    uint32_t gsa = smem_u32(&groups[threadIdx.x / G]);
+    asm volatile("" : "+r"(gsa));
+    GroupSmem<R, G, BS> &gs = *(GroupSmem<R, G, BS> *)__cvta_shared_to_generic(gsa);
+    GroupScratch<R, G, false> &sc = gs.sc;
+    unsigned char *slot_base = ws + (size_t)(blockIdx.x * (PLAN_THREADS / G) + threadIdx.x / G) * L.slot_bytes;
+    asm volatile("" : "+l"(slot_base));
+    const Tree<R> T{slot_base, L, P.cap};
+#define BIN_COUNT(b) (BS ? (int)gs.bins[0][b] : T.count()[b])
+#define BIN_HEAD(b) (BS ? (int)gs.bins[1][b] : T.head()[b])
+#define BIN_TAIL(b) (BS ? (int)gs.bins[2][b] : T.tail()[b])
+#define SET_BIN_COUNT(b, v) do { if (BS) gs.bins[0][b] = (unsigned short)(v); else T.count()[b] = (v); } while (0)
+#define SET_BIN_HEAD(b, v) do { if (BS) gs.bins[1][b] = (unsigned short)(v); else T.head()[b] = (v); } while (0)
+#define SET_BIN_TAIL(b, v) do { if (BS) gs.bins[2][b] = (unsigned short)(v); else T.tail()[b] = (v); } while (0)
 
     for (;;) {
         long long q = 0;
@@ -176,8 +186,6 @@
         q = g.bcast(q, 0);
         if (q >= Q) break;
 
-        Stream<R> rng;
-        rng.key = stream_key(seeds[q]); rng.ext = nullptr; rng.n_ext = 0;
         const R sx = starts[5 * q], sy = starts[5 * q + 1], sth = starts[5 * q + 2], st = starts[5 * q + 3],
                 slen = starts[5 * q + 4];
         for (int b = g.gl; b < P.nb + 2; b += G) SET_BIN_COUNT(b, 0);
@@ -188,19 +196,21 @@
             Contrib c = point_contrib<R>(env, sx, sy, st, 0xffffffffu, env.H, env.classify(sx, sy));
             r0.self_s2 = (c.bin >= 0 && c.cell >= 0) ? A::mul(P.w3, env.probs[(size_t)c.bin * env.C + c.cell]) : (R)0;
             r0.self_hab = c.bin >= 0 ? c.hab : -1;
-            T.row[0] = r0;
-            if (pick_mode == 1 || pick_mode == 3) { T.nx[0] = sx; T.ny[0] = sy; }
+            T.row()[0] = r0;
+            if (pick_mode == 1 || pick_mode == 3) { T.nx()[0] = sx; T.ny()[0] = sy; }
         }
         g.sync();
-        if (g.gl == 0) { SET_BIN_HEAD(1, 0); SET_BIN_TAIL(1, 0); SET_BIN_COUNT(1, 1); T.pool[0] = 0; T.next[0] = -1; }
+        if (g.gl == 0) { SET_BIN_HEAD(1, 0); SET_BIN_TAIL(1, 0); SET_BIN_COUNT(1, 1); T.pool()[0] = 0; T.next()[0] = -1; }
         g.sync();
+        Stream<R> rng;
+        rng.key = stream_key(seeds[q]); rng.ext = nullptr; rng.n_ext = 0;
         int n_nodes = 1, n_chunks = 1;
         uint32_t ctr = 0, upos_mark = 0;
         int status = AUVRRT_ST_OK;
         int n_cost_evals = 0;
         unsigned n_waypoints = 0, n_prims = 0;
         R best_total = A::inf();
-        if (g.gl == 0) { BestPlan<R> b0; b0.c0 = b0.c1 = b0.c2 = b0.len = b0.t = (R)0; b0.node = -1; b0.iter = -1; best_s[threadIdx.x / G] = b0; }
+        if (g.gl == 0) { BestPlan<R> b0; b0.c0 = b0.c1 = b0.c2 = b0.len = b0.t = (R)0; b0.node = -1; b0.iter = -1; gs.best = b0; }
         int it = 0;
         int guard = 0;
         const int guard_max = (int)min(64LL * P.I + 1024, 2147483647LL);
@@ -219,7 +229,7 @@
                     const int i = i0 + g.gl;
                     bool in = false;
                     if (i < n_nodes) {
-                        const R qq = A::sq2(A::sub(smx, T.nx[i]), A::sub(smy, T.ny[i]));
+                        const R qq = A::sq2(A::sub(smx, T.nx()[i]), A::sub(smy, T.ny()[i]));
                         if (qq < bq) {
                             if (VERIFY) { R sd = A::sqrt(qq); if (sd < bs) { bs = sd; bi = i; } }
                             else { bs = qq; bi = i; }
@@ -243,7 +253,7 @@
                 }
                 const int nearest = bi;
                 g.sync();
-                if (T.row[nearest].t > P.max_traj) { upos_mark = ctr; continue; }
+                if (T.row()[nearest].t > P.max_traj) { upos_mark = ctr; continue; }
                 int pn = nlist;
                 for (int j = g.gl; j < nlist; j += G) if (near[j] == nearest) pn = j;
 #pragma unroll
@@ -259,7 +269,7 @@
                 NodeRow<R> pr;
                 pr.s2 = 0; pr.self_s2 = 0; pr.cnt = 0; pr.mask = 0ull; pr.self_hab = -1; pr.t = 0;
                 if (pidx >= 0) {
-                    pr = T.row[pidx];
+                    pr = T.row()[pidx];
                     if (!(pr.t > P.max_traj))
                         dubins_edge_eval<R>(env, P, pr.x, pr.y, pr.th, pr.t, pr.len, smx, smy, smth, true, nullptr, 0, de);
                 }
@@ -304,8 +314,8 @@
                         nr.x = de.x; nr.y = de.y; nr.th = de.th; nr.t = de.t; nr.len = de.len; nr.parent = bp; nr.ctr = ctr0;
                         nr.s2 = pre_s2; nr.cnt = pre_cnt; nr.mask = pre_mask; nr.self_s2 = de.self_s2; nr.self_hab = de.self_hab;
                         nr.born = it;
-                        T.row[id] = nr;
-                        T.nx[id] = de.x; T.ny[id] = de.y;
+                        T.row()[id] = nr;
+                        T.nx()[id] = de.x; T.ny()[id] = de.y;
                     }
                     if (nt_ >= P.horizon) {
                         n_cost_evals++;
@@ -313,7 +323,7 @@
                             best_total = bt;
                             if (g.gl == bl) {
                                 BestPlan<R> b; b.c0 = c0; b.c1 = c1; b.c2 = c2; b.len = de.len; b.t = de.t; b.node = id; b.iter = it;
-                                best_s[threadIdx.x / G] = b;
+                                gs.best = b;
                             }
                         }
                     }
@@ -348,13 +358,13 @@
                 if (idx >= bincnt) { status = AUVRRT_ST_KEY_ERROR; break; }
                 int ch = BIN_HEAD(ran_bin);
 #pragma unroll 1
-                for (int hop = idx >> 5; hop > 0; hop--) ch = T.next[ch];
-                parent = T.pool[ch * 32 + (idx & 31)];
+                for (int hop = idx >> 5; hop > 0; hop--) ch = T.next()[ch];
+                parent = T.pool()[ch * 32 + (idx & 31)];
             } else if (pick_mode == 2) {
                 const R ran_time = uniform_ab<R>((R)0, P.ran_time_max, rng.u(ctr));
                 ctr += 1;
-                parent = closest_mps_time<R>(T.row, n_nodes, ran_time, P.plan_dt);
-                if (T.row[parent].t > P.max_traj) continue;
+                parent = closest_mps_time<R>(T.row(), n_nodes, ran_time, P.plan_dt);
+                if (T.row()[parent].t > P.max_traj) continue;
             } else {
                 R rx = uniform_ab<R>(env.minx, env.maxx, rng.u(ctr));
                 R ry = uniform_ab<R>(env.miny, env.maxy, rng.u(ctr + 1));
@@ -362,7 +372,7 @@
                 R bq = A::inf(), bs = A::inf();
                 int bi = 0x7fffffff;
                 for (int i = g.gl; i < n_nodes; i += G) {
-                    R qq = A::sq2(A::sub(rx, T.nx[i]), A::sub(ry, T.ny[i]));
+                    R qq = A::sq2(A::sub(rx, T.nx()[i]), A::sub(ry, T.ny()[i]));
                     if (qq < bq) {
                         if (VERIFY) { R s = A::sqrt(qq); if (s < bs) { bs = s; bi = i; } }
                         else { bs = qq; bi = i; }
@@ -376,10 +386,10 @@
                     if (os < bs || (os == bs && oi < bi)) { bs = os; bi = oi; }
                 }
                 parent = bi;
-                if (T.row[parent].t > P.max_traj) continue;
-            }
-            const NodeRow<R> pr = T.row[parent];
-            const R ppx = pr.x, ppy = pr.y, ppth = pr.th, ppt = pr.t, pplen = pr.len;
+                if (T.row()[parent].t > P.max_traj) continue;
+            }
+            const NodeRow<R> *prow = T.row() + parent;
+            const R ppx = prow->x, ppy = prow->y, ppth = prow->th, ppt = prow->t, pplen = prow->len;
             const uint32_t ctr0 = ctr;
 #if AUV_PLAN_PREFETCH
             int spec_parent = -1;
@@ -387,13 +397,13 @@
                 const int n_exp_now = (int)A::floor(uniform_ab<R>((R)0, P.sp.freq, rng.u(ctr)));
                 const uint32_t cn0 = ctr + 1u + 3u * (uint32_t)(n_exp_now > 0 ? n_exp_now : 0);
                 const int rb = (int)uniform_ab<R>((R)1, (R)(P.nb + 1), rng.u(cn0 + (uint32_t)g.gl));
-                const int cn = (rb >= 1 && rb <= P.nb) ? (int)s_count[rb] : 0;
+                const int cn = (rb >= 1 && rb <= P.nb) ? (int)gs.bins[0][rb] : 0;
                 const unsigned m = g.ballot(cn > 0);
                 if (m) {
                     const int f = __ffs(m) - 1;
                     const int sb = g.bcast(rb, f), sc_ = g.bcast(cn, f);
                     const int idx = (int)uniform_ab<R>((R)0, (R)sc_, rng.u(cn0 + (uint32_t)f + 1u));
-                    if (idx < 32 && idx < sc_) spec_parent = T.pool[(int)s_head[sb] * 32 + idx];
+                    if (idx < 32 && idx < sc_) spec_parent = T.pool()[(int)gs.bins[1][sb] * 32 + idx];
                 }
             }
 #endif
@@ -402,7 +412,7 @@
                                                            nullptr, 0, o);
 #if AUV_PLAN_PREFETCH
             if (ONE && BS && pick_mode == 0 && spec_parent >= 0 && g.gl < 2)
-                asm volatile("prefetch.global.L1 [%0];" ::"l"((const char *)&T.row[spec_parent] + 32 * g.gl));
+                asm volatile("prefetch.global.L1 [%0];" ::"l"((const char *)&T.row()[spec_parent] + 32 * g.gl));
 #endif
             ctr = o.ctr;
             n_waypoints += o.nwp; n_prims += o.n_exp;
@@ -415,21 +425,22 @@
             if (o.status != 0) { status = o.status; break; }
             if (o.safe) {
                 const int id = n_nodes++;
-                R pre_s2 = 0, self_s2n = 0;
-                uint32_t pre_cnt = 0; unsigned long long pre_mask = 0; int self_habn = -1;
+                const R pr_s2 = prow->s2, pr_self_s2 = prow->self_s2;
+                const uint32_t pr_cnt = prow->cnt;
+                const int ph = prow->self_hab;
+                const unsigned long long pr_mask = prow->mask;
+                const R pre_s2 = A::add(A::add(pr_s2, pr_self_s2), o.s2);
+                const uint32_t pre_cnt = pr_cnt + (ph >= 0 ? 1u : 0u) + o.cnt;
+                const unsigned long long pre_mask = pr_mask | (ph >= 0 ? (1ull << ph) : 0ull) | o.mask;
+                const R self_s2n = o.leaf_moved ? o.self_s2 : pr_self_s2;
+                const int self_habn = o.leaf_moved ? o.self_hab : ph;
                 if (g.gl == 0) {
-                    const int ph = pr.self_hab;
-                    pre_s2 = A::add(A::add(pr.s2, pr.self_s2), o.s2);
-                    pre_cnt = pr.cnt + (ph >= 0 ? 1u : 0u) + o.cnt;
-                    pre_mask = pr.mask | (ph >= 0 ? (1ull << ph) : 0ull) | o.mask;
-                    self_s2n = o.leaf_moved ? o.self_s2 : pr.self_s2;
-                    self_habn = o.leaf_moved ? o.self_hab : ph;
                     NodeRow<R> nr;
                     nr.x = o.x; nr.y = o.y; nr.th = o.th; nr.t = o.t; nr.len = o.len; nr.parent = parent; nr.ctr = ctr0;
                     nr.s2 = pre_s2; nr.cnt = pre_cnt; nr.mask = pre_mask; nr.self_s2 = self_s2n; nr.self_hab = self_habn;
                     nr.born = it;
-                    T.row[id] = nr;
-                    if (pick_mode == 1 || pick_mode == 3) { T.nx[id] = o.x; T.ny[id] = o.y; }
+                    T.row()[id] = nr;
+                    if (pick_mode == 1 || pick_mode == 3) { T.nx()[id] = o.x; T.ny()[id] = o.y; }
                 }
                 if (pick_mode != 2) {
                     R fd = floordiv_pos<R>(o.t, P.bin_interval);
@@ -451,37 +462,30 @@
                         if (g.gl == 0) {
                             int tl = reuse_head ? BIN_HEAD(bidx) : BIN_TAIL(bidx);
                             if (alloc) {
-                                T.next[nc] = -1;
-                                if (c == 0) SET_BIN_HEAD(bidx, nc); else T.next[tl] = nc;
+                                T.next()[nc] = -1;
+                                if (c == 0) SET_BIN_HEAD(bidx, nc); else T.next()[tl] = nc;
                                 tl = nc;
                             }
                             SET_BIN_TAIL(bidx, tl);
-                            T.pool[tl * 32 + (c & 31)] = id;
+                            T.pool()[tl * 32 + (c & 31)] = id;
                             SET_BIN_COUNT(bidx, c + 1);
                         }
                     }
                 }
-                status = g.bcast(status, 0);
                 if (status != AUVRRT_ST_OK) break;
                 if (o.t >= P.horizon) {
-                    R tot_s2 = 0, c0 = 0, c1 = 0, c2 = 0, total = 0;
-                    if (g.gl == 0) {
-                        uint32_t cnt = pre_cnt + (self_habn >= 0 ? 1u : 0u);
-                        unsigned long long mk = pre_mask | (self_habn >= 0 ? (1ull << self_habn) : 0ull);
-                        tot_s2 = A::add(pre_s2, self_s2n);
-                        c1 = A::mul(P.w2, (R)cnt);
-                        c2 = tot_s2;
-                        if (o.t > (R)0) { c1 = A::div(c1, o.t); c2 = A::div(c2, o.t); }
-                        if (env.H != 0) c0 = A::div(A::mul(P.w1, (R)__popcll(mk)), (R)env.H);
-                        total = py_sum3p<R>(c0, c1, c2);
-                    }
-                    total = g.bcast(total, 0);
+                    const uint32_t cnt = pre_cnt + (self_habn >= 0 ? 1u : 0u);
+                    const unsigned long long mk = pre_mask | (self_habn >= 0 ? (1ull << self_habn) : 0ull);
+                    R c0 = 0, c1 = A::mul(P.w2, (R)cnt), c2 = A::add(pre_s2, self_s2n);
+                    if (o.t > (R)0) { c1 = A::div(c1, o.t); c2 = A::div(c2, o.t); }
+                    if (env.H != 0) c0 = A::div(A::mul(P.w1, (R)__popcll(mk)), (R)env.H);
+                    const R total = py_sum3p<R>(c0, c1, c2);
                     n_cost_evals++;
                     if (total < best_total) {
                         best_total = total;
                         if (g.gl == 0) {
                             BestPlan<R> b; b.c0 = c0; b.c1 = c1; b.c2 = c2; b.len = o.len; b.t = o.t; b.node = id; b.iter = it;
-                            best_s[threadIdx.x / G] = b;
+                            gs.best = b;
                         }
                     }
                 }
@@ -491,7 +495,8 @@
             upos_mark = ctr;
         }
         g.sync();
-        const BestPlan<R> best = best_s[threadIdx.x / G];
+        rng.key = stream_key(seeds[q]);
+        const BestPlan<R> best = gs.best;
         const int best_node = best.node, best_iter = best.iter;
         const R best_c[4] = {best_total, best.c0, best.c1, best.c2}, best_len = best.len, best_t = best.t;
         if (status == AUVRRT_ST_OK && best_node < 0) status = AUVRRT_ST_NO_PATH;
@@ -499,19 +504,19 @@
         if (best_node < 0 && chain_out)
             for (int k = g.gl; k < P.chain_cap; k += G) chain_out[(size_t)q * P.chain_cap + k] = 0u;
         if (best_node >= 0) {
-            for (int n = best_node; T.row[n].parent >= 0; n = T.row[n].parent) depth++;
+            for (int n = best_node; T.row()[n].parent >= 0; n = T.row()[n].parent) depth++;
             uint32_t *chain = chain_out ? chain_out + (size_t)q * P.chain_cap : nullptr;
             if (depth > P.chain_cap && chain) { if (status == AUVRRT_ST_OK) status = AUVRRT_ST_OVERFLOW; }
             if (chain && g.gl == 0) {
                 int n = best_node;
-                for (int k = depth - 1; k >= 0; k--) { if (k < P.chain_cap) chain[k] = (uint32_t)n; n = T.row[n].parent; }
+                for (int k = depth - 1; k >= 0; k--) { if (k < P.chain_cap) chain[k] = (uint32_t)n; n = T.row()[n].parent; }
             }
             g.sync();
             if (path_out && P.path_cap > 0 && chain && depth <= P.chain_cap) {
                 R *rows = path_out + (size_t)q * P.path_cap * 6;
                 for (int e = 0; e < depth; e++) {
                     const int id = (int)chain[e];
-                    const NodeRow<R> pn = T.row[T.row[id].parent];
+                    const NodeRow<R> pn = T.row()[T.row()[id].parent];
                     if (g.gl == 0 && n_path < P.path_cap) {
                         R *w = rows + 6 * (size_t)n_path;
                         w[0] = pn.x; w[1] = pn.y; w[2] = pn.th; w[3] = (pick_mode == 3 && pn.parent >= 0) ? P.vel : (R)0;
@@ -522,7 +527,7 @@
                     if (pick_mode == 3) {
                         if (g.gl == 0) {
                             R smx, smy, smth;
-                            dubins_sample_at<R>(env, rng, T.row[id].ctr, smx, smy, smth);
+                            dubins_sample_at<R>(env, rng, T.row()[id].ctr, smx, smy, smth);
                             DubinsEdge<R> de;
                             dubins_edge_eval<R>(env, P, pn.x, pn.y, pn.th, pn.t, pn.len, smx, smy, smth, false,
                                                 rows + 6 * (size_t)(n_path < P.path_cap ? n_path : 0), room, de);
@@ -531,14 +536,14 @@
                         continue;
                     }
                     EdgeOut<R> o;
-                    eval_edge<R, G, false, false, true>(g, sc, env, rng, T.row[id].ctr, P.sp, pn.x, pn.y, pn.th,
+                    eval_edge<R, G, false, false, true>(g, sc, env, rng, T.row()[id].ctr, P.sp, pn.x, pn.y, pn.th,
                                                         pn.t, pn.len, (R)0, 0,
                                                         rows + 6 * (size_t)(n_path < P.path_cap ? n_path : 0), room, o);
                     n_path += o.nwp - 1;
                 }
                 if (g.gl == 0 && n_path < P.path_cap) {
                     R *w = rows + 6 * (size_t)n_path;
-                    const NodeRow<R> bn = T.row[best_node];
+                    const NodeRow<R> bn = T.row()[best_node];
                     w[0] = bn.x; w[1] = bn.y; w[2] = bn.th; w[3] = (pick_mode == 3 && bn.parent >= 0) ? P.vel : (R)0;
                     w[4] = bn.t; w[5] = bn.len;
                 }
@@ -547,7 +552,7 @@
             }
             g.sync();
             if (chain && g.gl == 0)
-                for (int k = 0; k < depth && k < P.chain_cap; k++) chain[k] = T.row[chain[k]].ctr;
+                for (int k = 0; k < depth && k < P.chain_cap; k++) chain[k] = T.row()[chain[k]].ctr;
             if (chain) for (int k = depth + g.gl; k < P.chain_cap; k += G) chain[k] = 0u;
         }
         if (g.gl == 0) {
@@ -664,7 +669,12 @@
     auvrrt_plan_trace_t tr;
     if (trace) tr = *trace; else { tr.parent = nullptr; tr.safe = nullptr; tr.nwp = nullptr; tr.leaf = nullptr; tr.upos = nullptr; }
     EnvBlob<R> b = env_blob<R>(env);
-    k_plan<R, G, BS, MODE, ONE><<<grid, PlanCta<R, G>::T, smem, s>>>(b.blob, b.hot_bytes, b.total_bytes, mode, starts, seeds, (long long)Q, P, L,
+    const EnvHeader &hd = sizeof(R) == 4 ? env->h32 : env->h64;
+    EnvView<R> ev;
+    ev.bind_header(hd, b.blob, b.blob);
+    ev.bind_grid_header(hd, b.blob, b.blob);
+    ev.bin_lo = hd.T > 0 ? (R)env->h_bins[0] : (R)1; ev.bin_hi = hd.T > 0 ? (R)env->h_bins[2 * hd.T - 1] : (R)0;
+    k_plan<R, G, BS, MODE, ONE><<<grid, PlanCta<R, G>::T, smem, s>>>(b.blob, b.hot_bytes, b.total_bytes, mode, ev, starts, seeds, (long long)Q, P, L,
                                                   (unsigned char *)workspace + 256, (unsigned long long *)workspace,
                                                   records, chain, path, tr);
     AUV_LAUNCH_CHECK2();
@@ -684,7 +694,9 @@
             const bool fits = PlanCta<R, G>::T >= 896
                                   ? (env->h32.gnx > 0 && env->h32.total_bytes + 16 + env->h32.gnx * env->h32.gny * 4 + 16 <= 180 * 1024)
                                   : env->h32.hot_bytes + 16 <= 24 * 1024;
-            if (p->freq <= (double)G && bs && fits && !getenv("AUVRRT_PLAN_STAGE_KB"))
+            const float fq = (float)p->freq;
+            const bool one_chunk = p->freq <= (double)G && floorf(fmaf(fq, 2.0f - 0x1p-23f, -fq)) <= (float)(G - 1);
+            if (one_chunk && bs && fits && !getenv("AUVRRT_PLAN_STAGE_KB"))
                 return launch_plan_gb<R, G, true, 0, true>(AUV_PLAN_ARGS);
             return bs ? launch_plan_gb<R, G, true, 0, false>(AUV_PLAN_ARGS) : launch_plan_gb<R, G, false, 0, false>(AUV_PLAN_ARGS);
         }
```
